# muhammadhasyim/cav-hoomd

Measured on AMD Instinct MI355X. Metric: cavity_force_evals_per_sec, higher is better.
Workload: dtype f64; 1 GPU; config3/config5: 1e6 diatomic particles + photon, finite-q start, g=1e-3, omegac=2000cm^-1; one independent replica per GPU (seed = rank+1); ring of 7 trajectory frames (HBM-cold); N_particles=1000001, frames=7, primed_frames=7, replicas=1, algorithmic_bytes_per_eval=92000092, layout=HOOMD AoS (Scalar4 pos/force, int3 image)

## Files before the change

### cav-hoomd_amd/csrc/cavmd_capi.hip

```cpp
#include <hip/hip_runtime.h>
#include <hip/hip_ext.h>

#include <math.h>
#include <stdio.h>
#include <stdlib.h>
#include <string.h>

#include <algorithm>
#include <new>
#include <vector>

#include "cavmd.h"
#include "cavmd_kernels.hpp"
#include "cavmd_host_support.hpp"

using namespace cavmd;

namespace
{
constexpr int kReduceBlock = 256;
constexpr int kReduceUnroll = 2;
constexpr int kFinalizeBlock = 256;
constexpr int kMapBlock = 256;
constexpr int kMapUnroll = 4;
constexpr int kMaxBlocksPerCU = 16;
constexpr int kEventsPerSlot = 6;
constexpr int kProfileSlots = 512;
constexpr size_t kMaxSamples = 4096;
constexpr int kSmallBlock = 256;
constexpr int kSmallSystemMaxN = 1024;
constexpr size_t kNtStoreMinN = 200000;
constexpr size_t kChargeTemporalMaxN = 25000000;
constexpr int kPersistBlock = 256;
constexpr size_t kPersistMaxLds = 156 * 1024;
constexpr uint64_t kSuspendFirst = 1ull << 16, kSuspendMax = 1ull << 31, kSuspendForever = ~0ull;
constexpr size_t kPersistSharedLds = 76 * 1024;
constexpr unsigned kResultHistory = 64;
constexpr unsigned kResultHistoryMax = 16384;

static_assert(sizeof(cavmd_double4) == 32, "Scalar4 layout");
static_assert(sizeof(cavmd_int3) == 12, "int3 layout");
static_assert(sizeof(cavmd_params) == 32, "params layout");
static_assert(sizeof(cavmd_result) == 192, "result layout");

struct HostControl
{
    HostResult fixed;
    unsigned sync_error;
    unsigned pad[63];
};
}

struct cavmd_workspace
{
    int device = -1;
    int num_cu = 0;
    char arch[64] = {0};
    size_t max_N = 0;
    unsigned max_parts = 0;
    DeviceArray<double> d_part;
    DeviceArray<int> d_ipart;
    DeviceArray<cavmd_result> d_result;
    MappedBlock<HostResult> h_ring;
    unsigned ring_depth = kResultHistory;
    uint64_t history_first = 1;
    MappedBlock<HostControl> h_ctl;
    hipStream_t last_stream = nullptr;
    bool computed = false;
    uint64_t sequence = 0;
    int reduce_blocks_per_cu = 1;
    int map_blocks_per_cu = 2;
    int map_nt_store = -1;
    int reduce_nt_load = -1;
    int fused_finalize = 1;
    int map_reverse = -1;
    int small_system_max_n = kSmallSystemMaxN;
    int reduce_unroll = -1;
    int persistent = -1;
    int rho_lane_particle = -1;
    int persistent_lds_kb = 0;
    int persistent_balanced = -1;
    DeviceArray<unsigned long long> d_granules;
    DeviceArray<unsigned> d_epoch;
    int debug_spin_limit = 0;
    int debug_late_block = -1;
    int debug_late_ticks = 0;
    int debug_silent_block = -1;
    int debug_skip_publish = 0;
    MappedBlock<HostResult> h_scratch;
    uint64_t suspend_until = 0;
    uint64_t suspend_backoff = kSuspendFirst;
    bool sync_state_dirty = false;
    bool sync_timeout_seen = false;
    bool captured = false;
    uint64_t captured_from = 0;
    bool profiling = false;
    std::vector<hipEvent_t> events;
    int pending = 0;
    std::vector<unsigned> slot_mask;
    double acc_ms[3] = {0, 0, 0};
    uint64_t acc_launches = 0;
    std::vector<float> samples;
    size_t n_k = 0;
    unsigned n_chunks = 0;
    unsigned rho_blocks = 0;
    DeviceArray<double> d_kvec, d_rho_part, d_rho;
    PinnedBlock<double> h_rho;
    hipStream_t rho_stream = nullptr;
    bool rho_computed = false;
    int rho_last_mapping = -1;
    int rho_last_blocks = -1;
    DeviceArray<double> d_mode;
    MappedBlock<HostMode> h_mode;
    uint64_t mode_sequence = 0;
    DeviceArray<double> d_fm_part;
    MappedBlock<HostScalar> h_fm;
    uint64_t fm_sequence = 0;
    DeviceArray<unsigned> d_fm_ticket;
    DeviceArray<BussiDevice> d_bussi;
    MappedBlock<HostBussi> h_bussi;
    uint64_t bussi_sequence = 0;
    uint64_t bussi_refused_seen = 0;
    hipStream_t bussi_stream = nullptr;
    unsigned bussi_batches = 0;
    unsigned recorders = 0;
    unsigned field_recorders = 0;
};

namespace
{
struct DeviceGuard
{
    int prev = -1;
    bool switched = false;
    explicit DeviceGuard(int dev)
    {
        if (hipGetDevice(&prev) == hipSuccess && prev != dev)
        {
            switched = (hipSetDevice(dev) == hipSuccess);
        }
    }
    ~DeviceGuard()
    {
        if (switched)
            (void)hipSetDevice(prev);
    }
};

inline int hip_status(hipError_t e)
{
    return e == hipSuccess ? CAVMD_OK : (int)e;
}

#define CAVMD_HIP_TRY(expr)              \
    do                                   \
    {                                    \
        hipError_t _e = (expr);          \
        if (_e != hipSuccess)            \
            return (int)_e;              \
    } while (0)

DeviceParams derive(const cavmd_params* p)
{
    DeviceParams d;
    d.g = p->couplstr;
    d.K = p->K;
    d.gK = p->couplstr / p->K;
    d.g2K = p->couplstr * p->couplstr / p->K;
    return d;
}

bool params_ok(const cavmd_params* p)
{
    return p && isfinite(p->omegac) && isfinite(p->couplstr) && isfinite(p->K) && isfinite(p->phmass) && p->K != 0.0;
}

int drain_profile(cavmd_workspace* ws)
{
    for (int s = 0; s < ws->pending; ++s)
    {
        hipEvent_t* ev = &ws->events[kEventsPerSlot * s];
        const unsigned used = ws->slot_mask[s];
        float sample[3] = {0.f, 0.f, 0.f};
        for (int k = 0; k < 3; ++k)
        {
            if (!(used & (1u << k)))
                continue;
            CAVMD_HIP_TRY(hipEventSynchronize(ev[2 * k + 1]));
            float ms = 0.f;
            CAVMD_HIP_TRY(hipEventElapsedTime(&ms, ev[2 * k], ev[2 * k + 1]));
            ws->acc_ms[k] += (double)ms;
            sample[k] = ms;
        }
        ws->acc_launches += 1;
        if (ws->samples.size() >= 3 * kMaxSamples)
            ws->samples.erase(ws->samples.begin(), ws->samples.begin() + 3);
        ws->samples.insert(ws->samples.end(), sample, sample + 3);
    }
    ws->pending = 0;
    return CAVMD_OK;
}

void note_capture(cavmd_workspace* ws, hipStream_t stream)
{
    if (!ws->captured && stream_capturing(stream))
    {
        ws->captured = true;
        ws->captured_from = ws->sequence;
    }
}

constexpr bool kPersistentAuto = true;
constexpr bool kPersistentBalancedAuto = false;

unsigned grid_for(size_t work_items, unsigned tile, int num_cu, int blocks_per_cu)
{
    size_t tiles = (work_items + tile - 1) / tile;
    size_t cap = (size_t)num_cu * (size_t)blocks_per_cu;
    size_t g = tiles < cap ? tiles : cap;
    return (unsigned)(g ? g : 1);
}

constexpr int kScaleBlocksPerCu = 4;
constexpr size_t kTicketBytes = 128;

int ensure_scalar_scratch(cavmd_workspace* ws)
{
    if (ws->d_fm_part.ptr)
        return CAVMD_OK;
    DeviceArray<double> part;
    MappedBlock<HostScalar> host;
    DeviceArray<unsigned> ticket;
    CAVMD_HIP_TRY(part.alloc(2 * (size_t)ws->max_parts + 1));
    CAVMD_HIP_TRY(host.alloc());
    CAVMD_HIP_TRY(ticket.alloc_zeroed(kTicketBytes / sizeof(unsigned)));
    ws->d_fm_part = std::move(part);
    ws->h_fm = std::move(host);
    ws->d_fm_ticket = std::move(ticket);
    return CAVMD_OK;
}

int wait_scalar(cavmd_workspace* ws, hipStream_t stream, double* out)
{
    const StampWait w = wait_for_stamp(&ws->h_fm.host->ready, ws->fm_sequence, stream);
    if (w.error != hipSuccess)
        return (int)w.error;
    if (!w.arrived)
    {
        (void)hipMemsetAsync(ws->d_fm_ticket.ptr, 0, kTicketBytes, stream);
        return (int)hipErrorLaunchFailure;
    }
    *out = ws->h_fm.host->value;
    return CAVMD_OK;
}

constexpr IntList<2, 1> kUnrolls;
constexpr IntList<0, 1, 2> kLoadPolicies;
constexpr IntList<2, 1, 0> kStorePolicies;

hipError_t allow_large_lds()
{
    hipError_t once = [] {
        hipError_t e = hipSuccess;
        const auto allow = [&e](auto kernel) {
            if (e == hipSuccess)
                e = hipFuncSetAttribute(reinterpret_cast<const void*>(kernel), hipFuncAttributeMaxDynamicSharedMemorySize,
                                        (int)kPersistMaxLds);
        };
        with_each_constant(kUnrolls, [&](auto u) {
            with_each_constant(kStorePolicies, [&](auto s) {
                allow(&cavity_persistent_kernel<kPersistBlock, decltype(u)::value, decltype(s)::value>);
            });
        });
#ifdef CAVMD_TEST_HOOKS
        with_each_constant(kUnrolls, [&](auto u) { allow(&cavity_persistent_kernel<kPersistBlock, decltype(u)::value, 0, true>); });
#endif
        return e;
    }();
    return once;
}

struct LaunchScope
{
    cavmd_workspace* ws;
    hipStream_t stream;
    hipEvent_t* ev = nullptr;
    unsigned used = 0;
    int status = CAVMD_OK;
    LaunchScope(cavmd_workspace* w, hipStream_t s) : ws(w), stream(s)
    {
        if (!ws->profiling)
            return;
        if (ws->pending == kProfileSlots)
            status = drain_profile(ws);
        if (status == CAVMD_OK)
            ev = &ws->events[kEventsPerSlot * ws->pending];
    }
    template <class K, class... Args>
    int launch_lds(int slot, size_t lds_bytes, K kernel, unsigned grid, unsigned block, Args... args)
    {
        if (ev)
        {
            hipExtLaunchKernelGGL(kernel, dim3(grid), dim3(block), lds_bytes, stream, ev[2 * slot], ev[2 * slot + 1], 0,
                                  args...);
            used |= 1u << slot;
        }
        else
            hipLaunchKernelGGL(kernel, dim3(grid), dim3(block), lds_bytes, stream, args...);
        return hip_status(hipGetLastError());
    }
    template <class K, class... Args>
    int launch(int slot, K kernel, unsigned grid, unsigned block, Args... args)
    {
        return launch_lds(slot, 0, kernel, grid, block, args...);
    }
    void commit()
    {
        if (ev)
        {
            ws->slot_mask[ws->pending] = used;
            ws->pending += 1;
        }
    }
};

enum class Layout
{
    aos,
    strided
};

enum class Path
{
    single_block,
    single_launch,
    two_launches,
    three_launches
};

struct EvalPlan
{
    Path path = Path::two_launches;
    Path multi_launch = Path::two_launches;
    int unroll = kReduceUnroll;
    unsigned g1 = 1, g2 = 1;
    int nt_load = 0;
    int nt_store = 0;
    unsigned lds_slots = 0;
    size_t lds_bytes = 0;
    bool balanced = false;
    bool map_reverse = false;
};

EvalPlan plan_evaluation(const cavmd_workspace& ws, size_t N, Layout layout)
{
    EvalPlan p;
    p.multi_launch = ws.fused_finalize ? Path::two_launches : Path::three_launches;
    p.path = p.multi_launch;
    if (layout == Layout::aos && ws.small_system_max_n > 0 && N <= (size_t)ws.small_system_max_n)
    {
        p.path = Path::single_block;
        return p;
    }
    p.unroll = kReduceUnroll;
    while (p.unroll > 1 && N / ((size_t)kReduceBlock * p.unroll) < (size_t)ws.num_cu * 5 / 4)
        p.unroll >>= 1;
    if (ws.reduce_unroll == 1 || ws.reduce_unroll == 2)
        p.unroll = ws.reduce_unroll;
    p.g1 = grid_for(N, kReduceBlock * p.unroll, ws.num_cu, ws.reduce_blocks_per_cu);
    if (layout == Layout::strided)
    {
        p.g2 = grid_for(N, kMapBlock * 4, ws.num_cu, ws.map_blocks_per_cu);
        return p;
    }
    p.g2 = grid_for(2 * N, kMapBlock * kMapUnroll, ws.num_cu, ws.map_blocks_per_cu);
    p.nt_store = ws.map_nt_store < 0 ? (N >= kNtStoreMinN ? 1 : 0) : ws.map_nt_store;
    p.nt_load = ws.reduce_nt_load < 0 ? (N <= kChargeTemporalMaxN ? 1 : 2) : ws.reduce_nt_load;
    p.map_reverse = ws.map_reverse < 0 ? (N > 2500000 && N <= 5000000) : (ws.map_reverse != 0);

    const size_t tile = (size_t)kReduceBlock * p.unroll;
    p.balanced = ws.persistent_balanced < 0 ? kPersistentBalancedAuto : (ws.persistent_balanced != 0);
    size_t slots;
    if (p.balanced)
    {
        const size_t units = (N + kWave - 1) / kWave;
        slots = (((units + p.g1 - 1) / p.g1) * kWave + tile - 1) / tile;
    }
    else
        slots = ((N + tile - 1) / tile + p.g1 - 1) / p.g1;
    size_t budget = kPersistMaxLds / (size_t)ws.reduce_blocks_per_cu - 1024;
    if (ws.persistent_lds_kb > 0 && (size_t)ws.persistent_lds_kb * 1024 < budget)
        budget = (size_t)ws.persistent_lds_kb * 1024;
    const size_t cap_slots = budget / (tile * sizeof(double));
    p.lds_slots = (unsigned)(slots < cap_slots ? slots : cap_slots);
    p.lds_bytes = p.lds_slots * tile * sizeof(double);
    const bool resident = p.g1 <= kMaxPersistGrid && ws.reduce_blocks_per_cu <= 4;
    if (resident
        && (ws.persistent > 0
            || (ws.persistent < 0 && slots <= cap_slots && p.lds_bytes <= kPersistSharedLds && kPersistentAuto)))
        p.path = Path::single_launch;
    return p;
}

int evaluation_enqueued(cavmd_workspace* ws, LaunchScope& ls, hipStream_t stream)
{
    ls.commit();
    ws->last_stream = stream;
    ws->computed = true;
    return CAVMD_OK;
}
}

extern "C"
{

cavmd_params cavmd_make_params(double omegac, double couplstr, double phmass)
{
    cavmd_params p;
    p.omegac = omegac;
    p.couplstr = couplstr;
    p.phmass = phmass;
    p.K = phmass * omegac * omegac;
    return p;
}

int cavmd_create(int device, size_t max_N, cavmd_workspace** out_ws)
{
    if (!out_ws)
        return CAVMD_ERR_INVALID_VALUE;
    *out_ws = nullptr;
    if (max_N > (size_t)INT_MAX)
        return CAVMD_ERR_CAPACITY;
    int count = 0;
    hipError_t e = hipGetDeviceCount(&count);
    if (e != hipSuccess || count <= 0)
        return CAVMD_ERR_NO_DEVICE;
    if (device < 0)
    {
        if (hipGetDevice(&device) != hipSuccess)
            return CAVMD_ERR_NO_DEVICE;
    }
    if (device >= count)
        return CAVMD_ERR_INVALID_VALUE;

    cavmd_workspace* ws = new (std::nothrow) cavmd_workspace();
    if (!ws)
        return (int)hipErrorOutOfMemory;
    ws->device = device;
    ws->max_N = max_N;
    if (const char* env = getenv("CAVMD_PERSISTENT"))
    {
        if (!strcmp(env, "0"))
            ws->persistent = 0;
        else if (!strcmp(env, "1"))
            ws->persistent = 1;
    }
    DeviceGuard guard(device);

    hipDeviceProp_t prop;
    e = hipGetDeviceProperties(&prop, device);
    if (e != hipSuccess)
    {
        delete ws;
        return (int)e;
    }
    ws->num_cu = prop.multiProcessorCount > 0 ? prop.multiProcessorCount : 256;
    strncpy(ws->arch, prop.gcnArchName, sizeof(ws->arch) - 1);
    ws->max_parts = (unsigned)(ws->num_cu * kMaxBlocksPerCU);

    e = ws->d_part.alloc((size_t)kNumPartDoubles * ws->max_parts);
    if (e == hipSuccess)
        e = ws->d_ipart.alloc((size_t)kNumPartInts * ws->max_parts);
    if (e == hipSuccess)
        e = ws->d_result.alloc_zeroed(1);
    if (e == hipSuccess)
        e = ws->d_granules.alloc_zeroed((size_t)2 * kGranulesPerRecord * kMaxPersistGrid);
    if (e == hipSuccess)
        e = ws->d_epoch.alloc(4);
    if (e == hipSuccess)
    {
        const unsigned init[4] = {1u, 0u, 0u, 0u};
        e = hipMemcpy(ws->d_epoch.ptr, init, sizeof(init), hipMemcpyHostToDevice);
    }
    if (e == hipSuccess)
        e = allow_large_lds();
    if (e == hipSuccess)
        e = ws->h_ring.alloc(ws->ring_depth);
    if (e == hipSuccess)
        e = ws->h_ctl.alloc();
    if (e != hipSuccess)
    {
        delete ws;
        return (int)e;
    }
    *out_ws = ws;
    return CAVMD_OK;
}

int cavmd_destroy(cavmd_workspace* ws)
{
    if (!ws)
        return CAVMD_OK;
    if (ws->bussi_batches != 0)
        return CAVMD_ERR_INVALID_VALUE;
    if (ws->recorders != 0)
        return CAVMD_ERR_INVALID_VALUE;
    if (ws->field_recorders != 0)
        return CAVMD_ERR_INVALID_VALUE;
    DeviceGuard guard(ws->device);
    for (hipEvent_t ev : ws->events)
        (void)hipEventDestroy(ev);
    delete ws;
    return CAVMD_OK;
}

namespace
{
inline HostResult* host_block(cavmd_workspace* ws)
{
#ifdef CAVMD_TEST_HOOKS
    if (ws->debug_skip_publish && ws->h_scratch.dev)
        return ws->h_scratch.dev;
#endif
    if (ws->captured)
        return &ws->h_ctl.dev->fixed;
    return ws->h_ring.dev + ws->sequence % ws->ring_depth;
}

inline HostResult* ring_slot(cavmd_workspace* ws, uint64_t s)
{
    return ws->h_ring.host + s % ws->ring_depth;
}

inline HostResult* last_block(cavmd_workspace* ws)
{
    if (ws->captured)
        return __atomic_load_n(&ws->h_ctl.host->fixed.ready, __ATOMIC_ACQUIRE) ? &ws->h_ctl.host->fixed
                                                                               : ring_slot(ws, ws->captured_from);
    return ring_slot(ws, ws->sequence);
}

unsigned consume_sync_timeout(cavmd_workspace* ws)
{
    if (!ws->h_ctl.host || !__atomic_load_n(&ws->h_ctl.host->sync_error, __ATOMIC_ACQUIRE))
        return 0;
    if (!stream_capturing(ws->last_stream))
        (void)hipStreamSynchronize(ws->last_stream);
    const unsigned verdict = __atomic_load_n(&ws->h_ctl.host->sync_error, __ATOMIC_ACQUIRE);
    __atomic_store_n(&ws->h_ctl.host->sync_error, 0u, __ATOMIC_RELEASE);
    ws->sync_timeout_seen = true;
    ws->sync_state_dirty = true;
    if (verdict == kSyncRepaired)
    {
        if (ws->sequence - ws->suspend_until > ws->suspend_backoff)
            ws->suspend_backoff = kSuspendFirst;
        ws->suspend_until = ws->sequence + ws->suspend_backoff;
        ws->suspend_backoff = ws->suspend_backoff * 8 < kSuspendMax ? ws->suspend_backoff * 8 : kSuspendMax;
        return kSyncRepaired;
    }
    ws->suspend_until = kSuspendForever;
    ws->computed = false;
    return kSyncFailed;
}
}

int cavmd_compute_hoomd(cavmd_workspace* ws, void* stream_, size_t N, const cavmd_double4* d_pos, const double* d_charge,
                        const cavmd_int3* d_image, double Lx, double Ly, double Lz, int L_typeid,
                        const cavmd_params* params, cavmd_double4* d_force)
{
    if (!ws || !d_pos || !d_charge || !d_image || !d_force || !params)
        return CAVMD_ERR_INVALID_VALUE;
    if (((uintptr_t)d_pos & 15) || ((uintptr_t)d_force & 15) || ((uintptr_t)d_charge & 7) || ((uintptr_t)d_image & 3))
        return CAVMD_ERR_INVALID_VALUE;
    if (N == 0)
        return CAVMD_OK;
    if (N > ws->max_N)
        return CAVMD_ERR_CAPACITY;
    if (!params_ok(params))
        return CAVMD_ERR_BAD_PARAMS;
    if (consume_sync_timeout(ws) == kSyncFailed)
        return CAVMD_ERR_SYNC_TIMEOUT;

    hipStream_t stream = (hipStream_t)stream_;
    DeviceGuard guard(ws->device);
    note_capture(ws, stream);
    LaunchScope ls(ws, stream);
    if (ls.status != CAVMD_OK)
        return ls.status;

    AosInput in;
    in.pos2 = reinterpret_cast<const v2d*>(d_pos);
    in.charge = d_charge;
    in.image = reinterpret_cast<const int*>(d_image);
    Partials part {ws->d_part.ptr, ws->d_ipart.ptr, ws->max_parts};
    const unsigned n = (unsigned)N;
    const DeviceParams dp = derive(params);
    v2d* force2 = reinterpret_cast<v2d*>(d_force);
    cavmd_result* const d_result = ws->d_result.ptr;
    int st;

    EvalPlan plan = plan_evaluation(*ws, N, Layout::aos);
    if (plan.path == Path::single_launch && ws->sequence < ws->suspend_until)
        plan.path = plan.multi_launch;

    if (plan.path == Path::single_block)
    {
        ws->sequence += 1;
        st = ls.launch(0, cavity_small_system_kernel<kSmallBlock>, 1u, kSmallBlock, in, n, Lx, Ly, Lz, dp, L_typeid,
                       ws->sequence, d_result, host_block(ws), force2);
        return st != CAVMD_OK ? st : evaluation_enqueued(ws, ls, stream);
    }

    if (plan.path == Path::single_launch)
    {
        if (ws->sync_state_dirty)
        {
            CAVMD_HIP_TRY(hipMemsetAsync(ws->d_granules.ptr, 0, sizeof(unsigned long long) * 2 * kGranulesPerRecord * kMaxPersistGrid, stream));
            CAVMD_HIP_TRY(hipMemsetAsync(ws->d_epoch.ptr + 1, 0, 2 * sizeof(unsigned), stream));
            ws->sync_state_dirty = false;
        }
        ws->sequence += 1;
        const AosInputT<2> inx {in.pos2, in.charge, in.image};
        const SyncState sync {ws->d_granules.ptr, ws->d_epoch.ptr,
                              ws->debug_spin_limit > 0 ? (unsigned)ws->debug_spin_limit : kSpinLimit, ws->debug_late_block,
                              (unsigned)ws->debug_late_ticks, ws->debug_silent_block, &ws->h_ctl.dev->sync_error};
        const auto launch = [&](auto kernel) {
            return ls.launch_lds(0, plan.lds_bytes, kernel, plan.g1, kPersistBlock, inx, n, Lx, Ly, Lz, dp, L_typeid, sync,
                                 ws->sequence, d_result, host_block(ws), force2, plan.lds_slots, plan.balanced);
        };
#ifdef CAVMD_TEST_HOOKS
        if (ws->debug_late_block >= 0 || ws->debug_silent_block >= 0)
            st = with_constant(kUnrolls, plan.unroll, [&](auto u) {
                return launch(&cavity_persistent_kernel<kPersistBlock, decltype(u)::value, 0, true>);
            });
        else
#endif
            st = with_constant(kUnrolls, plan.unroll, [&](auto u) {
                return with_constant(kStorePolicies, plan.nt_store, [&](auto s) {
                    return launch(&cavity_persistent_kernel<kPersistBlock, decltype(u)::value, decltype(s)::value>);
                });
            });
        return st != CAVMD_OK ? st : evaluation_enqueued(ws, ls, stream);
    }

    st = with_constant(kUnrolls, plan.unroll, [&](auto u) {
        return with_constant(kLoadPolicies, plan.nt_load, [&](auto nt) {
            using Input = AosInputT<decltype(nt)::value>;
            return ls.launch(0, &dipole_partials_kernel<Input, kReduceBlock, decltype(u)::value, false>, plan.g1, kReduceBlock,
                             Input {in.pos2, in.charge, in.image}, n, Lx, Ly, Lz, L_typeid, part);
        });
    });
    if (st != CAVMD_OK)
        return st;

    ws->sequence += 1;
    if (plan.path == Path::two_launches)
    {
        st = with_constant(kStorePolicies, plan.nt_store, [&](auto s) {
            return ls.launch(2, &force_map_aos_fused_kernel<kMapBlock, kMapUnroll, decltype(s)::value>, plan.g2, kMapBlock, in, n,
                             plan.g1, Lx, Ly, Lz, dp, L_typeid, part, ws->sequence, d_result, host_block(ws), force2,
                             plan.map_reverse);
        });
    }
    else
    {
        st = ls.launch(1, finalize_kernel<AosInput, kFinalizeBlock>, 1u, kFinalizeBlock, in, n, plan.g1, Lx, Ly, Lz, dp, part,
                       ws->sequence, d_result, host_block(ws));
        if (st != CAVMD_OK)
            return st;
        const cavmd_result* res = d_result;
        st = with_constant(IntList<1, 0> {}, plan.nt_store != 0, [&](auto nts) {
            return ls.launch(2, &force_map_aos_kernel<kMapBlock, kMapUnroll, decltype(nts)::value != 0>, plan.g2, kMapBlock,
                             d_charge, in.pos2, n, params->couplstr, L_typeid, res, force2);
        });
    }
    return st != CAVMD_OK ? st : evaluation_enqueued(ws, ls, stream);
}

int cavmd_compute_soa(cavmd_workspace* ws, void* stream_, size_t N, const double* d_position, size_t position_stride,
                      const int32_t* d_typeid, size_t typeid_stride, const int32_t* d_image, size_t image_stride,
                      const double* d_charge, size_t charge_stride, double Lx, double Ly, double Lz, int L_typeid,
                      const cavmd_params* params, double* d_force, size_t force_stride, double* d_potential_energy,
                      size_t potential_energy_stride)
{
    if (!ws || !d_position || !d_typeid || !d_image || !d_charge || !d_force || !params)
        return CAVMD_ERR_INVALID_VALUE;
    if (position_stride < 24 || typeid_stride < 4 || image_stride < 12 || charge_stride < 8 || force_stride < 24
        || (d_potential_energy && potential_energy_stride < 8))
        return CAVMD_ERR_INVALID_VALUE;
    if (((uintptr_t)d_position & 7) || (position_stride & 7) || ((uintptr_t)d_charge & 7) || (charge_stride & 7)
        || ((uintptr_t)d_force & 7) || (force_stride & 7) || ((uintptr_t)d_typeid & 3) || (typeid_stride & 3)
        || ((uintptr_t)d_image & 3) || (image_stride & 3)
        || (d_potential_energy && (((uintptr_t)d_potential_energy & 7) || (potential_energy_stride & 7))))
        return CAVMD_ERR_INVALID_VALUE;
    if (N == 0)
        return CAVMD_OK;
    if (N > ws->max_N)
        return CAVMD_ERR_CAPACITY;
    if (!params_ok(params))
        return CAVMD_ERR_BAD_PARAMS;

    {
        const char* p0 = reinterpret_cast<const char*>(d_position);
        const char* f0 = reinterpret_cast<const char*>(d_force);
        if (position_stride == 32 && typeid_stride == 32 && reinterpret_cast<const char*>(d_typeid) == p0 + 24
            && image_stride == 12 && charge_stride == 8 && force_stride == 32 && d_potential_energy
            && potential_energy_stride == 32 && reinterpret_cast<const char*>(d_potential_energy) == f0 + 24
            && !((uintptr_t)p0 & 15) && !((uintptr_t)f0 & 15))
        {
            return cavmd_compute_hoomd(ws, stream_, N, reinterpret_cast<const cavmd_double4*>(d_position), d_charge,
                                       reinterpret_cast<const cavmd_int3*>(d_image), Lx, Ly, Lz, L_typeid, params,
                                       reinterpret_cast<cavmd_double4*>(d_force));
        }
    }

    hipStream_t stream = (hipStream_t)stream_;
    DeviceGuard guard(ws->device);
    note_capture(ws, stream);
    LaunchScope ls(ws, stream);
    if (ls.status != CAVMD_OK)
        return ls.status;

    StridedInput in;
    in.pos = reinterpret_cast<const char*>(d_position);
    in.tid = reinterpret_cast<const char*>(d_typeid);
    in.img = reinterpret_cast<const char*>(d_image);
    in.chg = reinterpret_cast<const char*>(d_charge);
    in.pos_stride = position_stride;
    in.tid_stride = typeid_stride;
    in.img_stride = image_stride;
    in.chg_stride = charge_stride;
    Partials part {ws->d_part.ptr, ws->d_ipart.ptr, ws->max_parts};
    const unsigned n = (unsigned)N;
    const DeviceParams dp = derive(params);
    cavmd_result* const d_result = ws->d_result.ptr;

    const EvalPlan plan = plan_evaluation(*ws, N, Layout::strided);
    int st = with_constant(kUnrolls, plan.unroll, [&](auto u) {
        return ls.launch(0, &dipole_partials_kernel<StridedInput, kReduceBlock, decltype(u)::value, false>, plan.g1, kReduceBlock,
                         in, n, Lx, Ly, Lz, L_typeid, part);
    });
    if (st != CAVMD_OK)
        return st;
    ws->sequence += 1;
    char* f_out = reinterpret_cast<char*>(d_force);
    char* pe_out = reinterpret_cast<char*>(d_potential_energy);
    if (plan.path == Path::two_launches)
    {
        st = ls.launch(2, force_map_strided_fused_kernel<kMapBlock>, plan.g2, kMapBlock, in, n, plan.g1, Lx, Ly, Lz, dp, L_typeid,
                       part, ws->sequence, d_result, host_block(ws), f_out, force_stride, pe_out, potential_energy_stride);
    }
    else
    {
        st = ls.launch(1, finalize_kernel<StridedInput, kFinalizeBlock>, 1u, kFinalizeBlock, in, n, plan.g1, Lx, Ly, Lz, dp, part,
                       ws->sequence, d_result, host_block(ws));
        if (st != CAVMD_OK)
            return st;
        const cavmd_result* res = d_result;
        st = ls.launch(2, force_map_strided_kernel<kMapBlock>, plan.g2, kMapBlock, in, n, params->couplstr, L_typeid, res, f_out,
                       force_stride, pe_out, potential_energy_stride);
    }
    return st != CAVMD_OK ? st : evaluation_enqueued(ws, ls, stream);
}

int cavmd_result_read(cavmd_workspace* ws, cavmd_result* out)
{
    if (!ws || !out)
        return CAVMD_ERR_INVALID_VALUE;
    if (!ws->computed)
        return CAVMD_ERR_NOT_COMPUTED;
    DeviceGuard guard(ws->device);
    bool published = true;
    if (ws->captured)
    {
        CAVMD_HIP_TRY(hipDeviceSynchronize());
    }
    else
    {
        const StampWait w = wait_for_stamp(&ring_slot(ws, ws->sequence)->ready, ws->sequence, ws->last_stream);
        if (w.error != hipSuccess)
            return (int)w.error;
        published = w.arrived;
    }
    if (consume_sync_timeout(ws) == kSyncFailed)
        return CAVMD_ERR_SYNC_TIMEOUT;
    if (!published)
    {
        ws->computed = false;
        return (int)hipErrorLaunchFailure;
    }
    memcpy(out, &last_block(ws)->result, sizeof(cavmd_result));
    return CAVMD_OK;
}

int cavmd_energies(cavmd_workspace* ws, double out[3])
{
    if (!ws || !out)
        return CAVMD_ERR_INVALID_VALUE;
    if (!ws->computed)
    {
        out[0] = out[1] = out[2] = 0.0;
        return CAVMD_OK;
    }
    cavmd_result r;
    int st = cavmd_result_read(ws, &r);
    if (st != CAVMD_OK)
        return st;
    out[0] = r.energy[0];
    out[1] = r.energy[1];
    out[2] = r.energy[2];
    return CAVMD_OK;
}

int cavmd_last_sequence(cavmd_workspace* ws, uint64_t* out)
{
    if (!ws || !out)
        return CAVMD_ERR_INVALID_VALUE;
    *out = ws->sequence;
    return CAVMD_OK;
}

int cavmd_result_at(cavmd_workspace* ws, uint64_t sequence, cavmd_result* out)
{
    if (!ws || !out)
        return CAVMD_ERR_INVALID_VALUE;
    if (ws->sequence == 0)
        return CAVMD_ERR_NOT_COMPUTED;
    if (ws->captured)
        return CAVMD_ERR_INVALID_VALUE;
    const uint64_t last = ws->sequence;
    if (sequence == 0 || sequence > last)
        return CAVMD_ERR_INVALID_VALUE;
    if (sequence < ws->history_first || last - sequence >= ws->ring_depth)
        return CAVMD_ERR_EXPIRED;
    DeviceGuard guard(ws->device);
    const HostResult* h = ring_slot(ws, sequence);
    const StampWait w = wait_for_stamp(&h->ready, sequence, ws->last_stream, [&] {
        for (uint64_t j = sequence + 1; j <= last; ++j)
            if (__atomic_load_n(&ring_slot(ws, j)->ready, __ATOMIC_ACQUIRE) == j)
                return true;
        return false;
    });
    if (w.error != hipSuccess)
        return (int)w.error;
    if (!w.arrived)
    {
        const uint64_t failed = __atomic_load_n(&h->failed, __ATOMIC_ACQUIRE);
        return failed == ((sequence << 2) | kSyncFailed) ? CAVMD_ERR_SYNC_TIMEOUT : (int)hipErrorLaunchFailure;
    }
    memcpy(out, &h->result, sizeof(cavmd_result));
    return CAVMD_OK;
}

int cavmd_energies_at(cavmd_workspace* ws, uint64_t sequence, double out[3])
{
    if (!ws || !out)
        return CAVMD_ERR_INVALID_VALUE;
    cavmd_result r;
    const int st = cavmd_result_at(ws, sequence, &r);
    if (st != CAVMD_OK)
        return st;
    out[0] = r.energy[0];
    out[1] = r.energy[1];
    out[2] = r.energy[2];
    return CAVMD_OK;
}

int cavmd_result_device_ptr(cavmd_workspace* ws, const cavmd_result** out)
{
    if (!ws || !out)
        return CAVMD_ERR_INVALID_VALUE;
    *out = ws->d_result.ptr;
    return CAVMD_OK;
}

int cavmd_set_wavevectors(cavmd_workspace* ws, size_t n_k, const double* h_wavevectors)
{
    if (!ws || !h_wavevectors || n_k == 0 || n_k > (size_t)1 << 20)
        return CAVMD_ERR_INVALID_VALUE;
    DeviceGuard guard(ws->device);
    ws->d_kvec.free();
    ws->d_rho_part.free();
    ws->d_rho.free();
    ws->h_rho.free();
    ws->rho_computed = false;
    ws->n_k = 0;
    const unsigned n_chunks = (unsigned)((n_k + kWave - 1) / kWave);
    const unsigned rho_blocks = (unsigned)ws->num_cu * 4;
    DeviceArray<double> kvec, rho_part, rho;
    PinnedBlock<double> h_rho;
    CAVMD_HIP_TRY(kvec.alloc(3 * n_k));
    CAVMD_HIP_TRY(rho_part.alloc(2 * kWave * (size_t)n_chunks * rho_blocks));
    CAVMD_HIP_TRY(rho.alloc(2 * n_k));
    CAVMD_HIP_TRY(h_rho.alloc(2 * n_k));
    CAVMD_HIP_TRY(hipMemcpy(kvec.ptr, h_wavevectors, sizeof(double) * 3 * n_k, hipMemcpyHostToDevice));
    ws->d_kvec = std::move(kvec);
    ws->d_rho_part = std::move(rho_part);
    ws->d_rho = std::move(rho);
    ws->h_rho = std::move(h_rho);
    ws->n_k = n_k;
    ws->n_chunks = n_chunks;
    ws->rho_blocks = rho_blocks;
    return CAVMD_OK;
}

int cavmd_density_field(cavmd_workspace* ws, void* stream_, size_t N, const double* d_position, size_t position_stride)
{
    if (!ws || !d_position || position_stride < 24 || (position_stride & 7) || ((uintptr_t)d_position & 7))
        return CAVMD_ERR_INVALID_VALUE;
    if (ws->n_k == 0)
        return CAVMD_ERR_NOT_COMPUTED;
    if (N > (size_t)INT_MAX)
        return CAVMD_ERR_CAPACITY;
    hipStream_t stream = (hipStream_t)stream_;
    DeviceGuard guard(ws->device);
    constexpr int kBlock = 1024;
    const size_t tiles = (N + kWave - 1) / kWave;
    unsigned gb;
    int lp = ws->rho_lane_particle;
    if (lp < 0)
        lp = (ws->n_k * 4 < (size_t)ws->n_chunks * kWave * 3) ? 3 : 0;
    if (lp)
    {
        constexpr int kLpBlock = 256;
        size_t g = (tiles + (kLpBlock / kWave) - 1) / (kLpBlock / kWave);
        if (g > ws->rho_blocks)
            g = ws->rho_blocks;
        gb = (unsigned)(g ? g : 1);
        with_constant(IntList<25, 10, 5> {}, lp == 1 ? 25 : lp == 2 ? 10 : 5, [&](auto kc) {
            constexpr int KC = decltype(kc)::value;
            hipLaunchKernelGGL((density_partials_lp_kernel<kLpBlock, KC>), dim3(gb, (unsigned)((ws->n_k + KC - 1) / KC)),
                               dim3(kLpBlock), 0, stream, reinterpret_cast<const char*>(d_position), position_stride, (unsigned)N,
                               ws->d_kvec.ptr, (unsigned)ws->n_k, make_sincos_coef(), ws->d_rho_part.ptr);
        });
// ... 93 lines not shown
                       reinterpret_cast<const v2d*>(d_net_force), reinterpret_cast<const v2d*>(d_vel), (unsigned)N,
                       ws->d_fm_part.ptr, ws->d_fm_ticket.ptr, d_out, ws->h_fm.dev, ws->fm_sequence);
    CAVMD_HIP_TRY(hipGetLastError());
    return wait_scalar(ws, stream, out);
}

int cavmd_kinetic_energy(cavmd_workspace* ws, void* stream_, const cavmd_double4* d_vel, const uint32_t* d_members,
                         size_t n_members, double* out)
{
    if (!ws || !d_vel || !out || ((uintptr_t)d_vel & 15) || ((uintptr_t)d_members & 3))
        return CAVMD_ERR_INVALID_VALUE;
    if (n_members > (size_t)INT_MAX)
        return CAVMD_ERR_CAPACITY;
    if (n_members == 0)
    {
        *out = 0.0;
        return CAVMD_OK;
    }
    hipStream_t stream = (hipStream_t)stream_;
    DeviceGuard guard(ws->device);
    {
        const int st0 = ensure_scalar_scratch(ws);
        if (st0 != CAVMD_OK)
            return st0;
    }
    constexpr int kBlock = 256, kUnroll = 4;
    const unsigned g = grid_for(n_members, kBlock * kUnroll, ws->num_cu, 1);
    double* d_out = ws->d_fm_part.ptr + 2 * (size_t)ws->max_parts;
    ws->fm_sequence += 1;
    hipLaunchKernelGGL((kinetic_fused_kernel<kBlock, kUnroll>), dim3(g), dim3(kBlock), 0, stream,
                       reinterpret_cast<const v2d*>(d_vel), d_members, (unsigned)n_members, ws->d_fm_part.ptr,
                       ws->d_fm_ticket.ptr, d_out, ws->h_fm.dev, ws->fm_sequence);
    CAVMD_HIP_TRY(hipGetLastError());
    return wait_scalar(ws, stream, out);
}

int cavmd_scale_velocities(cavmd_workspace* ws, void* stream_, cavmd_double4* d_vel, const uint32_t* d_members,
                           size_t n_members, double alpha)
{
    if (!ws || !d_vel || ((uintptr_t)d_vel & 15) || ((uintptr_t)d_members & 3))
        return CAVMD_ERR_INVALID_VALUE;
    if (n_members > (size_t)INT_MAX)
        return CAVMD_ERR_CAPACITY;
    if (n_members == 0)
        return CAVMD_OK;
    hipStream_t stream = (hipStream_t)stream_;
    DeviceGuard guard(ws->device);
    constexpr int kBlock = 256, kUnroll = 4;
    const unsigned g = grid_for(n_members, kBlock * kUnroll, ws->num_cu, kScaleBlocksPerCu);
    hipLaunchKernelGGL((scale_velocities_kernel<kBlock, kUnroll>), dim3(g), dim3(kBlock), 0, stream, reinterpret_cast<v2d*>(d_vel),
                       d_members, (unsigned)n_members, alpha);
    return hip_status(hipGetLastError());
}

int cavmd_bussi_rescale_factor(double K, double degrees_of_freedom, double deltaT, double set_T, double tau,
                               double normal_variate, double gamma_variate, double* alpha)
{
    if (!alpha)
        return CAVMD_ERR_INVALID_VALUE;
    const double c = (tau != 0.0) ? exp(-deltaT / tau) : 0.0;
    *alpha = bussi_alpha_from_c(K, degrees_of_freedom, c, set_T, normal_variate, gamma_variate);
    return CAVMD_OK;
}

int cavmd_bussi_step(cavmd_bussi_reservoir* state, double K_translational, double dof_translational, double K_rotational,
                     double dof_rotational, double deltaT, double set_T, double tau, const double variates[4],
                     double factors[2])
{
    if (!state || !variates || !factors)
        return CAVMD_ERR_INVALID_VALUE;
    if (deltaT == 0.0)
    {
        factors[0] = factors[1] = 1.0;
        return CAVMD_OK;
    }
    if ((dof_translational != 0 && K_translational == 0) || (dof_rotational != 0 && K_rotational == 0))
        return CAVMD_ERR_BAD_PARAMS;
    double at = 1.0, ar = 1.0;
    (void)cavmd_bussi_rescale_factor(K_translational, dof_translational, deltaT, set_T, tau, variates[0], variates[1], &at);
    (void)cavmd_bussi_rescale_factor(K_rotational, dof_rotational, deltaT, set_T, tau, variates[2], variates[3], &ar);
    const double delta_t = K_translational * (1.0 - at * at);
    const double delta_r = K_rotational * (1.0 - ar * ar);
    state->reservoir_translational += delta_t;
    state->reservoir_rotational += delta_r;
    state->instantaneous_translational = delta_t;
    state->instantaneous_rotational = delta_r;
    factors[0] = at;
    factors[1] = ar;
    return CAVMD_OK;
}

namespace
{
int ensure_bussi_state(cavmd_workspace* ws)
{
    if (ws->d_bussi.ptr)
        return CAVMD_OK;
    DeviceArray<BussiDevice> state;
    MappedBlock<HostBussi> host;
    CAVMD_HIP_TRY(state.alloc_zeroed(1));
    CAVMD_HIP_TRY(host.alloc());
    ws->d_bussi = std::move(state);
    ws->h_bussi = std::move(host);
    return CAVMD_OK;
}
}

int cavmd_bussi_step_device(cavmd_workspace* ws, void* stream_, cavmd_double4* d_vel, const uint32_t* d_members,
                            size_t n_members, double dof_translational, double deltaT, double set_T, double tau,
                            double normal_variate, double gamma_variate)
{
    if (!ws || !d_vel || ((uintptr_t)d_vel & 15) || ((uintptr_t)d_members & 3))
        return CAVMD_ERR_INVALID_VALUE;
    if (n_members > (size_t)INT_MAX)
        return CAVMD_ERR_CAPACITY;
    hipStream_t stream = (hipStream_t)stream_;
    if (capture_state(stream) != Capture::none)
        return CAVMD_ERR_INVALID_VALUE;
    if (deltaT == 0.0 || n_members == 0)
        return CAVMD_OK;
    DeviceGuard guard(ws->device);
    {
        int st0 = ensure_scalar_scratch(ws);
        if (st0 == CAVMD_OK)
            st0 = ensure_bussi_state(ws);
        if (st0 != CAVMD_OK)
            return st0;
    }
    constexpr int kBlock = 256, kUnroll = 4;
    BussiStepArgs a;
    a.dof = dof_translational;
    a.c = (tau != 0.0) ? exp(-deltaT / tau) : 0.0;
    a.set_T = set_T;
    a.normal_variate = normal_variate;
    a.gamma_variate = gamma_variate;
    const unsigned g = grid_for(n_members, kBlock * kUnroll, ws->num_cu, 1);
    ws->bussi_sequence += 1;
    ws->bussi_stream = stream;
    hipLaunchKernelGGL((kinetic_partials_kernel<kBlock, kUnroll>), dim3(g), dim3(kBlock), 0, stream,
                       reinterpret_cast<const v2d*>(d_vel), d_members, (unsigned)n_members, ws->d_fm_part.ptr);
    CAVMD_HIP_TRY(hipGetLastError());
    const unsigned g2 = grid_for(n_members, kBlock * kUnroll, ws->num_cu, kScaleBlocksPerCu);
    hipLaunchKernelGGL((bussi_rescale_fused_kernel<kBlock, kUnroll>), dim3(g2), dim3(kBlock), 0, stream,
                       reinterpret_cast<v2d*>(d_vel), d_members, (unsigned)n_members, ws->d_fm_part.ptr, g, a, ws->d_bussi.ptr,
                       ws->h_bussi.dev, ws->bussi_sequence);
    return hip_status(hipGetLastError());
}

int cavmd_bussi_device_read(cavmd_workspace* ws, cavmd_bussi_device_state* out)
{
    if (!ws || !out)
        return CAVMD_ERR_INVALID_VALUE;
    memset(out, 0, sizeof(*out));
    if (!ws->d_bussi.ptr || ws->bussi_sequence == 0)
        return CAVMD_OK;
    DeviceGuard guard(ws->device);
    const StampWait w = wait_for_stamp(&ws->h_bussi.host->ready, ws->bussi_sequence, ws->bussi_stream);
    if (w.error != hipSuccess)
        return (int)w.error;
    if (!w.arrived)
        return (int)hipErrorLaunchFailure;
    const BussiDevice s = ws->h_bussi.host->state;
    out->reservoir_translational = s.reservoir;
    out->instantaneous_translational = s.instantaneous;
    out->last_alpha = s.alpha;
    out->last_kinetic_energy = s.kinetic;
    out->steps = s.steps;
    out->refused = s.errors;
    if (s.errors != ws->bussi_refused_seen)
    {
        ws->bussi_refused_seen = s.errors;
        return CAVMD_ERR_BAD_PARAMS;
    }
    return CAVMD_OK;
}

int cavmd_bussi_device_reset(cavmd_workspace* ws, void* stream_)
{
    if (!ws)
        return CAVMD_ERR_INVALID_VALUE;
    if (!ws->d_bussi.ptr)
        return CAVMD_OK;
    hipStream_t stream = (hipStream_t)stream_;
    DeviceGuard guard(ws->device);
    cavmd_bussi_device_state unused;
    const int st = cavmd_bussi_device_read(ws, &unused);
    if (st != CAVMD_OK && st != CAVMD_ERR_BAD_PARAMS)
        return st;
    CAVMD_HIP_TRY(hipMemsetAsync(ws->d_bussi.ptr, 0, sizeof(BussiDevice), stream));
    memset(&ws->h_bussi.host->state, 0, sizeof(BussiDevice));
    ws->bussi_refused_seen = 0;
    return CAVMD_OK;
}

int cavmd_profile_enable(cavmd_workspace* ws, int on)
{
    if (!ws)
        return CAVMD_ERR_INVALID_VALUE;
    DeviceGuard guard(ws->device);
    if (on && ws->events.empty())
    {
        ws->events.resize(kEventsPerSlot * kProfileSlots);
        ws->slot_mask.assign(kProfileSlots, 0);
        for (size_t i = 0; i < ws->events.size(); ++i)
        {
            hipError_t e = hipEventCreate(&ws->events[i]);
            if (e != hipSuccess)
            {
                for (size_t j = 0; j < i; ++j)
                    (void)hipEventDestroy(ws->events[j]);
                ws->events.clear();
                return (int)e;
            }
        }
    }
    if (!on && ws->pending)
    {
        int st = drain_profile(ws);
        if (st != CAVMD_OK)
            return st;
    }
    ws->profiling = on != 0;
    return CAVMD_OK;
}

int cavmd_profile_read(cavmd_workspace* ws, double ms[3], uint64_t* launches)
{
    if (!ws || !ms || !launches)
        return CAVMD_ERR_INVALID_VALUE;
    DeviceGuard guard(ws->device);
    int st = drain_profile(ws);
    if (st != CAVMD_OK)
        return st;
    for (int k = 0; k < 3; ++k)
    {
        ms[k] = ws->acc_ms[k];
        ws->acc_ms[k] = 0.0;
    }
    *launches = ws->acc_launches;
    ws->acc_launches = 0;
    ws->samples.clear();
    return CAVMD_OK;
}

int cavmd_profile_samples(cavmd_workspace* ws, double* out, size_t cap, size_t* n)
{
    if (!ws || !out || !n)
        return CAVMD_ERR_INVALID_VALUE;
    DeviceGuard guard(ws->device);
    int st = drain_profile(ws);
    if (st != CAVMD_OK)
        return st;
    const size_t have = ws->samples.size() / 3;
    const size_t take = have < cap ? have : cap;
    const size_t first = have - take;
    for (size_t i = 0; i < 3 * take; ++i)
        out[i] = (double)ws->samples[3 * first + i];
    *n = take;
    return CAVMD_OK;
}

namespace
{
int resize_history(cavmd_workspace* ws, unsigned depth)
{
    if (stream_capturing(ws->last_stream))
        return CAVMD_ERR_INVALID_VALUE;
    DeviceGuard guard(ws->device);
    if (ws->sequence)
        CAVMD_HIP_TRY(hipStreamSynchronize(ws->last_stream));
    MappedBlock<HostResult> ring;
    CAVMD_HIP_TRY(ring.alloc(depth));
    const uint64_t keep = ws->captured ? ws->captured_from : ws->sequence;
    if (keep)
        memcpy(ring.host + keep % depth, ring_slot(ws, keep), sizeof(HostResult));
    ws->h_ring = std::move(ring);
    ws->ring_depth = depth;
    ws->history_first = ws->sequence ? ws->sequence : 1;
    return CAVMD_OK;
}

struct TunableRow
{
    const char* name;
    int cavmd_workspace::*member;
    int lo, hi;
};
const TunableRow kTunables[] = {
    {"reduce_blocks_per_cu", &cavmd_workspace::reduce_blocks_per_cu, 1, kMaxBlocksPerCU},
    {"map_blocks_per_cu", &cavmd_workspace::map_blocks_per_cu, 1, kMaxBlocksPerCU},
    {"map_nt_store", &cavmd_workspace::map_nt_store, -1, 2},
    {"reduce_nt_load", &cavmd_workspace::reduce_nt_load, -1, 2},
    {"fused_finalize", &cavmd_workspace::fused_finalize, 0, 1},
    {"map_reverse", &cavmd_workspace::map_reverse, -1, 1},
    {"small_system_max_n", &cavmd_workspace::small_system_max_n, 0, 1 << 20},
    {"rho_lane_particle", &cavmd_workspace::rho_lane_particle, -1, 3},
    {"persistent_lds_kb", &cavmd_workspace::persistent_lds_kb, 0, 156},
    {"persistent_balanced", &cavmd_workspace::persistent_balanced, -1, 1},
#ifdef CAVMD_TEST_HOOKS
    {"debug_spin_limit", &cavmd_workspace::debug_spin_limit, 0, INT_MAX},
    {"debug_late_block", &cavmd_workspace::debug_late_block, -1, (int)kMaxPersistGrid - 1},
    {"debug_late_ticks", &cavmd_workspace::debug_late_ticks, 0, 100000000},
    {"debug_silent_block", &cavmd_workspace::debug_silent_block, -1, (int)kMaxPersistGrid - 1},
#endif
};

const TunableRow* find_tunable(const char* name)
{
    for (const TunableRow& row : kTunables)
        if (!strcmp(name, row.name))
            return &row;
    return nullptr;
}
}

int cavmd_set_tunable(cavmd_workspace* ws, const char* name, int value)
{
    if (!ws || !name)
        return CAVMD_ERR_INVALID_VALUE;
    if (const TunableRow* row = find_tunable(name))
    {
        if (value < row->lo || value > row->hi)
            return CAVMD_ERR_INVALID_VALUE;
        ws->*(row->member) = value;
        return CAVMD_OK;
    }
    if (!strcmp(name, "result_history"))
    {
        if (value < 2 || value > (int)kResultHistoryMax)
            return CAVMD_ERR_INVALID_VALUE;
        return resize_history(ws, (unsigned)value);
    }
    if (!strcmp(name, "persistent"))
    {
        if (value < -1 || value > 1)
            return CAVMD_ERR_INVALID_VALUE;
        ws->persistent = value;
        ws->suspend_until = 0;
        ws->suspend_backoff = kSuspendFirst;
        return CAVMD_OK;
    }
    if (!strcmp(name, "reduce_unroll"))
    {
        if (value != -1 && value != 1 && value != 2)
            return CAVMD_ERR_INVALID_VALUE;
        ws->reduce_unroll = value;
        return CAVMD_OK;
    }
#ifdef CAVMD_TEST_HOOKS
    if (!strcmp(name, "debug_suspend_first"))
    {
        if (value < 1)
            return CAVMD_ERR_INVALID_VALUE;
        ws->suspend_backoff = (uint64_t)value;
        return CAVMD_OK;
    }
    if (!strcmp(name, "debug_skip_publish"))
    {
        if (value < 0 || value > 1)
            return CAVMD_ERR_INVALID_VALUE;
        if (value && !ws->h_scratch.host)
        {
            DeviceGuard guard(ws->device);
            CAVMD_HIP_TRY(ws->h_scratch.alloc());
        }
        ws->debug_skip_publish = value;
        return CAVMD_OK;
    }
#endif
    if (!strcmp(name, "sync_timeout_seen"))
    {
#ifdef CAVMD_TEST_HOOKS
        if (value < 0 || value > 2)
            return CAVMD_ERR_INVALID_VALUE;
        if (value)
            __atomic_store_n(&ws->h_ctl.host->sync_error, value == 2 ? kSyncRepaired : kSyncFailed, __ATOMIC_RELEASE);
        else
            ws->sync_timeout_seen = false;
#else
        if (value != 0)
            return CAVMD_ERR_INVALID_VALUE;
        ws->sync_timeout_seen = false;
#endif
        return CAVMD_OK;
    }
    return CAVMD_ERR_INVALID_VALUE;
}

int cavmd_get_tunable(cavmd_workspace* ws, const char* name, int* value)
{
    if (!ws || !name || !value)
        return CAVMD_ERR_INVALID_VALUE;
    if (const TunableRow* row = find_tunable(name))
        *value = ws->*(row->member);
    else if (!strcmp(name, "result_history"))
        *value = (int)ws->ring_depth;
    else if (!strcmp(name, "persistent"))
        *value = ws->persistent;
    else if (!strcmp(name, "reduce_unroll"))
        *value = ws->reduce_unroll;
    else if (!strcmp(name, "sync_timeout_seen"))
        *value = ws->sync_timeout_seen ? 1 : 0;
    else if (!strcmp(name, "persistent_suspended"))
        *value = ws->suspend_until == kSuspendForever ? 2 : (ws->sequence < ws->suspend_until ? 1 : 0);
    else if (!strcmp(name, "rho_last_mapping"))
        *value = ws->rho_last_mapping;
    else if (!strcmp(name, "rho_last_blocks"))
        *value = ws->rho_last_blocks;
#ifdef CAVMD_TEST_HOOKS
    else if (!strcmp(name, "debug_skip_publish"))
        *value = ws->debug_skip_publish;
    else if (!strcmp(name, "test_hooks"))
        *value = 1;
#else
    else if (!strcmp(name, "test_hooks"))
        *value = 0;
#endif
    else
        return CAVMD_ERR_INVALID_VALUE;
    return CAVMD_OK;
}

int cavmd_device_info(cavmd_workspace* ws, int* device, int* compute_units, char* arch_name, size_t arch_name_len)
{
    if (!ws)
        return CAVMD_ERR_INVALID_VALUE;
    if (device)
        *device = ws->device;
    if (compute_units)
        *compute_units = ws->num_cu;
    if (arch_name && arch_name_len)
    {
        strncpy(arch_name, ws->arch, arch_name_len - 1);
        arch_name[arch_name_len - 1] = 0;
    }
    return CAVMD_OK;
}

const char* cavmd_error_string(int status)
{
    switch (status)
    {
    case CAVMD_OK:
        return "success";
    case CAVMD_ERR_INVALID_VALUE:
        return "invalid value (null or misaligned pointer, bad stride or size)";
    case CAVMD_ERR_NO_DEVICE:
        return "no HIP device available (this library has no CPU fallback)";
    case CAVMD_ERR_CAPACITY:
        return "N exceeds the workspace capacity";
    case CAVMD_ERR_BAD_PARAMS:
        return "bad cavity parameters (K == 0 or non-finite)";
    case CAVMD_ERR_NOT_COMPUTED:
        return "no evaluation has been enqueued on this workspace yet";
    case CAVMD_ERR_EXPIRED:
        return "that evaluation's result slot has been reused: read it sooner or raise the \"result_history\" tunable";
    case CAVMD_ERR_SYNC_TIMEOUT:
        return "a single-launch evaluation was starved (its workgroups were not resident together) and could not be completed; "
               "forces of that evaluation are NaN";
    default:
        break;
    }
    if (status > 0)
        return hipGetErrorString((hipError_t)status);
    return "unknown cavmd status";
}

int cavmd_version(void)
{
    return CAVMD_VERSION_MAJOR * 1000 + CAVMD_VERSION_MINOR;
}

}

#include "cavmd_item_table.hpp"

namespace
{
constexpr int kBatchBlock = kSmallBlock;
constexpr size_t kBatchRingMaxBytes = (size_t)64 << 20;
static_assert(sizeof(cavmd_batch_item) == 128, "batch item layout");

BatchRow batch_row(const cavmd_batch_item& it)
{
    BatchRow r;
    memset(&r, 0, sizeof(r));
    r.pos2 = reinterpret_cast<const v2d*>(it.d_pos);
    r.charge = it.d_charge;
    r.image = reinterpret_cast<const int*>(it.d_image);
    r.force2 = reinterpret_cast<v2d*>(it.d_force);
    r.Lx = it.Lx; r.Ly = it.Ly; r.Lz = it.Lz;
    if (it.N)
        r.prm = derive(&it.params);
    r.N = it.N;
    r.L_typeid = it.L_typeid;
    return r;
}
}

struct cavmd_batch : ItemTable<cavmd_batch_item, BatchRow>
{
    unsigned depth = 0;
    DeviceArray<cavmd_result> d_result;
    MappedBlock<HostResult> h_ring;
    uint64_t sequence = 0;
    bool captured = false;

    cavmd_batch() : ItemTable(cavmd_batch_item_check, [](const cavmd_batch_item& it) { return it.N; }, batch_row) {}
};

namespace
{
inline const HostResult* batch_slot(const cavmd_batch* b, uint64_t s)
{
    return b->h_ring.host + (s % b->depth) * b->n;
}
}

extern "C"
{

int cavmd_batch_item_check(const cavmd_batch_item* it)
{
    if (!it)
        return CAVMD_ERR_INVALID_VALUE;
    for (int k = 0; k < 4; ++k)
        if (it->reserved[k] != 0)
            return CAVMD_ERR_INVALID_VALUE;
    if (it->N != 0 && (!it->d_pos || !it->d_charge || !it->d_image || !it->d_force))
        return CAVMD_ERR_INVALID_VALUE;
    if (((uintptr_t)it->d_pos & 15) || ((uintptr_t)it->d_force & 15) || ((uintptr_t)it->d_charge & 7)
        || ((uintptr_t)it->d_image & 3))
        return CAVMD_ERR_INVALID_VALUE;
    if (it->N == 0)
        return CAVMD_OK;
    if (it->N > CAVMD_BATCH_MAX_ITEM_N)
        return CAVMD_ERR_CAPACITY;
    if (!params_ok(&it->params))
        return CAVMD_ERR_BAD_PARAMS;
    return CAVMD_OK;
}

int cavmd_batch_create(cavmd_workspace* ws, size_t n_items, const cavmd_batch_item* h_items, int history_depth,
                       cavmd_batch** out)
{
    if (!out)
        return CAVMD_ERR_INVALID_VALUE;
    *out = nullptr;
    if (!ws || !h_items || n_items == 0 || n_items > CAVMD_BATCH_MAX_ITEMS || history_depth < 2
        || history_depth > (int)kResultHistoryMax)
        return CAVMD_ERR_INVALID_VALUE;
    const int st = check_items(h_items, n_items, cavmd_batch_item_check);
    if (st != CAVMD_OK)
        return st;
    const size_t ring_blocks = (size_t)history_depth * n_items;
    if (ring_blocks * sizeof(HostResult) > kBatchRingMaxBytes)
        return CAVMD_ERR_CAPACITY;

    cavmd_batch* b = new (std::nothrow) cavmd_batch();
    if (!b)
        return (int)hipErrorOutOfMemory;
    b->adopt(ws->device, h_items, n_items);
    b->depth = (unsigned)history_depth;

    DeviceGuard guard(b->device);
    hipError_t e = b->upload();
    if (e == hipSuccess)
        e = b->d_result.alloc_zeroed(n_items);
    if (e == hipSuccess)
        e = b->h_ring.alloc(ring_blocks);
    if (e != hipSuccess)
    {
        cavmd_batch_destroy(b);
        return (int)e;
    }
    *out = b;
    return CAVMD_OK;
}

int cavmd_batch_destroy(cavmd_batch* b)
{
    if (!b)
        return CAVMD_OK;
    DeviceGuard guard(b->device);
    b->quiesce_and_free();
    delete b;
    return CAVMD_OK;
}

int cavmd_batch_set_items(cavmd_batch* b, size_t first, size_t count, const cavmd_batch_item* h_items)
{
    return b ? b->set_items(first, count, h_items) : CAVMD_ERR_INVALID_VALUE;
}

int cavmd_batch_compute(cavmd_batch* b, void* stream_)
{
    if (!b)
        return CAVMD_ERR_INVALID_VALUE;
    hipStream_t stream = (hipStream_t)stream_;
    DeviceGuard guard(b->device);
    if (!b->captured && stream_capturing(stream))
        b->captured = true;
    b->sequence += 1;
    HostResult* host = b->h_ring.dev + (b->sequence % b->depth) * b->n;
    hipLaunchKernelGGL(cavity_batch_kernel<kBatchBlock>, dim3((unsigned)b->n), dim3(kBatchBlock), 0, stream, b->d_rows,
                       b->d_order, b->sequence, b->d_result.ptr, host);
// ... 688 lines not shown
```

### cav-hoomd_amd/csrc/cavmd_force_kernels.hpp

```cpp
#pragma once

#include "cavmd_reduce.hpp"

#pragma clang fp contract(off)

namespace cavmd
{

template <int NT>
struct AosInputT
{
    const v2d* __restrict__ pos2;
    const double* __restrict__ charge;
    const int* __restrict__ image;

    struct Raw
    {
        v2d xy, zw;
        double c;
        int ix, iy, iz;
    };
    __device__ __forceinline__ Raw load(size_t i) const
    {
        Raw r;
// ... 5 lines not shown
            r.c = (NT == 2) ? __builtin_nontemporal_load(charge + i) : charge[i];
            r.ix = __builtin_nontemporal_load(im + 0);
            r.iy = __builtin_nontemporal_load(im + 1);
            r.iz = __builtin_nontemporal_load(im + 2);
        }
        else
        {
            r.xy = pos2[2 * i];
            r.zw = pos2[2 * i + 1];
            r.c = charge[i];
            r.ix = im[0];
            r.iy = im[1];
            r.iz = im[2];
        }
        return r;
    }
    static __device__ __forceinline__ double x(const Raw& r) { return r.xy.x; }
    static __device__ __forceinline__ double y(const Raw& r) { return r.xy.y; }
    static __device__ __forceinline__ double z(const Raw& r) { return r.zw.x; }
    static __device__ __forceinline__ int tag(const Raw& r) { return __double2loint(r.zw.y); }
};
typedef AosInputT<0> AosInput;

struct StridedInput
{
    const char* __restrict__ pos;
    const char* __restrict__ tid;
    const char* __restrict__ img;
    const char* __restrict__ chg;
    size_t pos_stride, tid_stride, img_stride, chg_stride;

    struct Raw
    {
        double px, py, pz, c;
        int ix, iy, iz, t;
    };
    __device__ __forceinline__ Raw load(size_t i) const
    {
        Raw r;
        const double* p = reinterpret_cast<const double*>(pos + i * pos_stride);
        r.px = __builtin_nontemporal_load(p + 0);
        r.py = __builtin_nontemporal_load(p + 1);
        r.pz = __builtin_nontemporal_load(p + 2);
        r.c = *reinterpret_cast<const double*>(chg + i * chg_stride);
        const int* im = reinterpret_cast<const int*>(img + i * img_stride);
        r.ix = __builtin_nontemporal_load(im + 0);
        r.iy = __builtin_nontemporal_load(im + 1);
        r.iz = __builtin_nontemporal_load(im + 2);
        r.t = __builtin_nontemporal_load(reinterpret_cast<const int*>(tid + i * tid_stride));
        return r;
    }
    static __device__ __forceinline__ double x(const Raw& r) { return r.px; }
    static __device__ __forceinline__ double y(const Raw& r) { return r.py; }
    static __device__ __forceinline__ double z(const Raw& r) { return r.pz; }
    static __device__ __forceinline__ int tag(const Raw& r) { return r.t; }
};

struct DeviceParams
{
    double g;
    double K;
    double gK;
    double g2K;
};

struct PhotonRow
{
    double x, y, z;
    int ix, iy, iz;
};
template <class Input>
__device__ __forceinline__ PhotonRow photon_row(const Input& in, size_t i)
{
    const typename Input::Raw r = in.load(i);
    PhotonRow p;
    p.x = Input::x(r); p.y = Input::y(r); p.z = Input::z(r);
    p.ix = r.ix; p.iy = r.iy; p.iz = r.iz;
    return p;
}

struct Partials
{
    double* d;
    int* i;
    unsigned stride;
};

template <class Input, int UNROLL>
struct TileRegs
{
    typename Input::Raw raw[UNROLL];
};

template <class Input, int BLOCK, int UNROLL>
__device__ __forceinline__ void tile_load(const Input& in, size_t base, TileRegs<Input, UNROLL>& r)
{
#pragma unroll
    for (int u = 0; u < UNROLL; ++u)
        r.raw[u] = in.load(base + (size_t)u * BLOCK);
}

template <class Input, int BLOCK, int UNROLL>
__device__ __forceinline__ void tile_accumulate(const TileRegs<Input, UNROLL>& r, size_t base, double Lx, double Ly,
                                                double Lz, int L_typeid, Accum& acc)
{
    bool isL[UNROLL];
    bool any = false;
#pragma unroll
    for (int u = 0; u < UNROLL; ++u)
    {
        isL[u] = (Input::tag(r.raw[u]) == L_typeid);
        any = any || isL[u];
    }
    if (!__any(any))
    {
#pragma unroll
        for (int u = 0; u < UNROLL; ++u)
        {
            const double c = r.raw[u].c;
            dd_acc(acc.hx, acc.lx, c * (Input::x(r.raw[u]) + (double)r.raw[u].ix * Lx));
            dd_acc(acc.hy, acc.ly, c * (Input::y(r.raw[u]) + (double)r.raw[u].iy * Ly));
            dd_acc(acc.hz, acc.lz, c * (Input::z(r.raw[u]) + (double)r.raw[u].iz * Lz));
        }
    }
    else
    {
#pragma unroll
        for (int u = 0; u < UNROLL; ++u)
        {
            const double rx = Input::x(r.raw[u]) + (double)r.raw[u].ix * Lx;
            const double ry = Input::y(r.raw[u]) + (double)r.raw[u].iy * Ly;
            const double rz = Input::z(r.raw[u]) + (double)r.raw[u].iz * Lz;
            acc.add((unsigned)(base + (size_t)u * BLOCK), rx, ry, rz, r.raw[u].c, Input::tag(r.raw[u]), L_typeid);
        }
    }
}

template <class Input, int BLOCK, int UNROLL, bool PIPE>
__global__ __launch_bounds__(BLOCK) void dipole_partials_kernel(Input in, unsigned N, double Lx, double Ly, double Lz,
                                                                int L_typeid, Partials part)
{
    constexpr unsigned TILE = BLOCK * UNROLL;
    Accum acc;
    const unsigned full_tiles = N / TILE;
    const unsigned G = gridDim.x;
    if (!PIPE)
    {
        for (unsigned t = blockIdx.x; t < full_tiles; t += G)
        {
            const size_t base = (size_t)t * TILE + threadIdx.x;
            TileRegs<Input, UNROLL> A;
            tile_load<Input, BLOCK, UNROLL>(in, base, A);
            __builtin_amdgcn_sched_barrier(0);
            tile_accumulate<Input, BLOCK, UNROLL>(A, base, Lx, Ly, Lz, L_typeid, acc);
        }
    }
    else
    {
        TileRegs<Input, UNROLL> A, B;
        unsigned t = blockIdx.x;
        if (t < full_tiles)
            tile_load<Input, BLOCK, UNROLL>(in, (size_t)t * TILE + threadIdx.x, A);
        while (t < full_tiles)
        {
            if (t + G < full_tiles)
                tile_load<Input, BLOCK, UNROLL>(in, (size_t)(t + G) * TILE + threadIdx.x, B);
            __builtin_amdgcn_sched_barrier(0);
            tile_accumulate<Input, BLOCK, UNROLL>(A, (size_t)t * TILE + threadIdx.x, Lx, Ly, Lz, L_typeid, acc);
            t += G;
            if (t >= full_tiles)
                break;
            if (t + G < full_tiles)
                tile_load<Input, BLOCK, UNROLL>(in, (size_t)(t + G) * TILE + threadIdx.x, A);
            __builtin_amdgcn_sched_barrier(0);
            tile_accumulate<Input, BLOCK, UNROLL>(B, (size_t)t * TILE + threadIdx.x, Lx, Ly, Lz, L_typeid, acc);
            t += G;
        }
    }
    if (blockIdx.x == full_tiles % G)
    {
        const size_t base = (size_t)full_tiles * TILE + threadIdx.x;
#pragma unroll
        for (int u = 0; u < UNROLL; ++u)
        {
            const size_t i = base + (size_t)u * BLOCK;
            if (i < N)
            {
                const typename Input::Raw r = in.load(i);
                const double rx = Input::x(r) + (double)r.ix * Lx;
                const double ry = Input::y(r) + (double)r.iy * Ly;
                const double rz = Input::z(r) + (double)r.iz * Lz;
                acc.add((unsigned)i, rx, ry, rz, r.c, Input::tag(r), L_typeid);
            }
        }
    }
    acc = block_reduce<BLOCK>(acc);
    if (threadIdx.x == 0)
    {
        const unsigned b = blockIdx.x, s = part.stride;
        part.d[0 * s + b] = acc.hx; part.d[1 * s + b] = acc.lx;
        part.d[2 * s + b] = acc.hy; part.d[3 * s + b] = acc.ly;
        part.d[4 * s + b] = acc.hz; part.d[5 * s + b] = acc.lz;
        part.d[6 * s + b] = acc.sx; part.d[7 * s + b] = acc.sy; part.d[8 * s + b] = acc.sz;
        part.i[0 * s + b] = acc.lmin;
        part.i[1 * s + b] = acc.lcnt;
    }
}

struct Scalars
{
    double d[3], dlo[3], q[3], Dq[2], e[3], f[3], dtot[3];
    int photon, nL;
};

template <class Input>
__device__ __forceinline__ Scalars scalars_from_total(Accum acc, const PhotonRow guess, const Input& in,
                                                      unsigned N, double Lx, double Ly, double Lz,
                                                      const DeviceParams& prm, bool want_energies)
{
    Scalars sc;
    dd_norm(acc.hx, acc.lx);
    dd_norm(acc.hy, acc.ly);
    if (want_energies)
        dd_norm(acc.hz, acc.lz);
    double dx = acc.hx, dy = acc.hy, dz = acc.hz;
    sc.dtot[0] = sc.dtot[1] = sc.dtot[2] = 0.0;
    if (want_energies)
    {
        double th = acc.hx, tl = acc.lx;
        dd_acc(th, tl, acc.sx);
        sc.dtot[0] = th + tl;
        th = acc.hy; tl = acc.ly;
        dd_acc(th, tl, acc.sy);
        sc.dtot[1] = th + tl;
        th = acc.hz; tl = acc.lz;
        dd_acc(th, tl, acc.sz);
        sc.dtot[2] = th + tl;
    }
    const int photon = (acc.lmin == INT_MAX) ? -1 : acc.lmin;
    const double g = prm.g, K = prm.K;
    double qx = 0.0, qy = 0.0, qz = 0.0, eh = 0.0, ec = 0.0, ed = 0.0, Dqx = 0.0, Dqy = 0.0, fx = 0.0, fy = 0.0, fz = 0.0;
    if (threadIdx.x == 0)
    {
        if (photon >= 0)
        {
            double px = guess.x, py = guess.y, pz = guess.z;
            int pix = guess.ix, piy = guess.iy, piz = guess.iz;
            if ((unsigned)photon != N - 1)
            {
                const PhotonRow r = photon_row(in, (size_t)photon);
                px = r.x; py = r.y; pz = r.z;
                pix = r.ix; piy = r.iy; piz = r.iz;
            }
            qx = px + (double)pix * Lx;
            qy = py + (double)piy * Ly;
            qz = pz + (double)piz * Lz;
            if (acc.lcnt > 1)
            {
                const double pc = in.load((size_t)photon).c;
                dx += acc.sx - pc * qx;
                dy += acc.sy - pc * qy;
                dz += acc.sz - pc * qz;
            }
            if (want_energies)
            {
                eh = 0.5 * K * (qx * qx + qy * qy + qz * qz);
                ec = g * (dx * qx + dy * qy + 0.0 * 0.0);
                ed = 0.5 * prm.g2K * (dx * dx + dy * dy + 0.0 * 0.0);
            }
            Dqx = qx + prm.gK * dx;
            Dqy = qy + prm.gK * dy;
            fx = -K * qx - g * dx;
            fy = -K * qy - g * dy;
            fz = -K * qz - g * 0.0;
        }
        else
        {
            dx = dy = dz = 0.0;
            acc.lx = acc.ly = acc.lz = 0.0;
        }
    }
    CAVMD_STAMP(4);
    sc.d[0] = dx; sc.d[1] = dy; sc.d[2] = dz;
    sc.dlo[0] = acc.lx; sc.dlo[1] = acc.ly; sc.dlo[2] = acc.lz;
    sc.q[0] = qx; sc.q[1] = qy; sc.q[2] = qz;
    sc.Dq[0] = Dqx; sc.Dq[1] = Dqy;
    sc.e[0] = eh; sc.e[1] = ec; sc.e[2] = ed;
    sc.f[0] = fx; sc.f[1] = fy; sc.f[2] = fz;
    sc.photon = photon;
    sc.nL = acc.lcnt;
    return sc;
}

template <class Input, int BLOCK>
__device__ __forceinline__ Scalars reduce_partials_and_finalize(const Input& in, unsigned N, unsigned nparts, double Lx,
                                                                double Ly, double Lz, const DeviceParams& prm,
                                                                const Partials& part, bool want_energies)
{
    CAVMD_STAMP(0);
    const PhotonRow guess = photon_row(in, (size_t)(N - 1));

    Accum acc;
    const unsigned s = part.stride;
    constexpr int BATCH = 4;
    for (unsigned base = 0; base < nparts; base += BATCH * BLOCK)
    {
        Accum o[BATCH];
#pragma unroll
        for (int j = 0; j < BATCH; ++j)
        {
            const unsigned p = base + j * BLOCK + threadIdx.x;
            if (p < nparts)
            {
                o[j].hx = part.d[0 * s + p]; o[j].lx = part.d[1 * s + p];
                o[j].hy = part.d[2 * s + p]; o[j].ly = part.d[3 * s + p];
                o[j].hz = part.d[4 * s + p]; o[j].lz = part.d[5 * s + p];
                o[j].sx = part.d[6 * s + p]; o[j].sy = part.d[7 * s + p]; o[j].sz = part.d[8 * s + p];
                o[j].lmin = part.i[0 * s + p];
                o[j].lcnt = part.i[1 * s + p];
            }
        }
#pragma unroll
        for (int j = 0; j < BATCH; ++j)
            if (base + j * BLOCK < nparts)
                acc.merge(o[j]);
    }
    CAVMD_STAMP(1);
    if (BLOCK == 256 && nparts <= 256)
    {
        __shared__ double s_gd[16][kNumPartDoubles];
        __shared__ int s_gi[16][kNumPartInts];
        acc = row_fold16(acc);
        CAVMD_STAMP(2);
        if ((threadIdx.x & 15) == 0)
        {
            const int gidx = threadIdx.x >> 4;
            s_gd[gidx][0] = acc.hx; s_gd[gidx][1] = acc.lx; s_gd[gidx][2] = acc.hy; s_gd[gidx][3] = acc.ly;
            s_gd[gidx][4] = acc.hz; s_gd[gidx][5] = acc.lz; s_gd[gidx][6] = acc.sx; s_gd[gidx][7] = acc.sy;
            s_gd[gidx][8] = acc.sz;
            s_gi[gidx][0] = acc.lmin;
            s_gi[gidx][1] = acc.lcnt;
        }
        __syncthreads();
        if (threadIdx.x < kWave)
        {
            Accum o;
            if (threadIdx.x < (nparts + 15) / 16)
            {
                const int gidx = threadIdx.x;
                o.hx = s_gd[gidx][0]; o.lx = s_gd[gidx][1]; o.hy = s_gd[gidx][2]; o.ly = s_gd[gidx][3];
                o.hz = s_gd[gidx][4]; o.lz = s_gd[gidx][5]; o.sx = s_gd[gidx][6]; o.sy = s_gd[gidx][7];
                o.sz = s_gd[gidx][8];
                o.lmin = s_gi[gidx][0];
                o.lcnt = s_gi[gidx][1];
            }
            Accum t;
            t.merge(o);
            acc = row_fold16(t);
        }
        CAVMD_STAMP(3);
    }
    else
        acc = block_reduce<BLOCK>(acc);
    return scalars_from_total<Input>(acc, guess, in, N, Lx, Ly, Lz, prm, want_energies);
}

__device__ __forceinline__ void write_result(cavmd_result* __restrict__ res, const Scalars& sc, unsigned N,
                                             unsigned nparts, uint64_t sequence)
{
#pragma unroll
    for (int k = 0; k < 3; ++k)
    {
        res->dipole[k] = sc.d[k];
        res->q[k] = sc.q[k];
        res->energy[k] = sc.e[k];
        res->photon_force[k] = sc.f[k];
        res->dipole_lo[k] = sc.dlo[k];
        res->total_dipole[k] = sc.dtot[k];
    }
    res->Dq[0] = sc.Dq[0];
    res->Dq[1] = sc.Dq[1];
    res->photon_idx = sc.photon;
    res->n_photon_typed = sc.nL;
    res->n_particles = N;
    res->n_partials = nparts;
    res->sequence = sequence;
    res->reserved = 0.0;
}

struct HostResult
{
    cavmd_result result;
    uint64_t ready;
    uint64_t failed;
    unsigned char pad[48];
};
static_assert(sizeof(HostResult) == 256, "one result slot = 256 bytes");
__device__ __forceinline__ void publish_to_host(HostResult* __restrict__ host, const Scalars& sc, unsigned N,
                                                unsigned nparts, uint64_t sequence)
{
    write_result(&host->result, sc, N, nparts, sequence);
    __hip_atomic_store(&host->ready, sequence, __ATOMIC_RELEASE, __HIP_MEMORY_SCOPE_SYSTEM);
}

template <class Input, int BLOCK>
__global__ __launch_bounds__(BLOCK) void finalize_kernel(Input in, unsigned N, unsigned nparts, double Lx, double Ly,
                                                         double Lz, DeviceParams prm, Partials part, uint64_t sequence,
                                                         cavmd_result* __restrict__ res, HostResult* __restrict__ res_host)
{
    const Scalars sc = reduce_partials_and_finalize<Input, BLOCK>(in, N, nparts, Lx, Ly, Lz, prm, part, true);
    if (threadIdx.x == 0)
    {
        write_result(res, sc, N, nparts, sequence);
        publish_to_host(res_host, sc, N, nparts, sequence);
    }
}

template <int NT>
__device__ __forceinline__ void store_chunk(v2d* p, v2d v)
{
    if (NT == 2)
    {
        asm volatile("global_store_dwordx4 %0, %1, off sc1\n\ts_nop 1" : : "v"(p), "v"(v) : "memory");
    }
    else if (NT == 1)
        __builtin_nontemporal_store(v, p);
    else
        *p = v;
}

struct MapScalars
{
    double Dqx, Dqy, Fx, Fy, Fz;
    int photon, nL;
};

template <int BLOCK, int UNROLL, int NT, bool PRE>
__device__ __forceinline__ void force_map_body(const MapScalars m, const double* __restrict__ charge,
                                               const v2d* __restrict__ pos2, unsigned N, double g, int L_typeid,
                                               v2d* __restrict__ force2, const double (&c_first)[UNROLL],
                                               bool reverse = false)
{
    constexpr unsigned TILE = BLOCK * UNROLL;
    const double ng = -g;
    const size_t nchunks = 2 * (size_t)N;
    const size_t pchunk = m.photon >= 0 ? 2 * (size_t)m.photon : ~(size_t)0;
    const unsigned full_tiles = (unsigned)(nchunks / TILE);
    const bool odd = threadIdx.x & 1;
    const v2d zero = {0.0, 0.0};

    if (m.photon < 0)
    {
        for (size_t k = (size_t)blockIdx.x * BLOCK + threadIdx.x; k < nchunks; k += (size_t)gridDim.x * BLOCK)
            store_chunk<NT>(force2 + k, zero);
        return;
    }

    if (m.nL <= 1)
    {
        const unsigned count = blockIdx.x < full_tiles ? (full_tiles - blockIdx.x + gridDim.x - 1) / gridDim.x : 0;
        for (unsigned j = 0; j < count; ++j)
        {
            const unsigned t = blockIdx.x + (reverse ? count - 1 - j : j) * gridDim.x;
            const size_t base = (size_t)t * TILE + threadIdx.x;
            double c[UNROLL];
            if (PRE && j == 0)
            {
#pragma unroll
                for (int u = 0; u < UNROLL; ++u)
                    c[u] = c_first[u];
            }
            else
            {
#pragma unroll
                for (int u = 0; u < UNROLL; ++u)
                    c[u] = charge[(base + (size_t)u * BLOCK) >> 1];
            }
#pragma unroll
            for (int u = 0; u < UNROLL; ++u)
            {
                const size_t k = base + (size_t)u * BLOCK;
                const double s = ng * c[u];
                v2d v = {s * m.Dqx, s * m.Dqy};
                v = odd ? zero : v;
                if ((k | 1) == (pchunk | 1))
                    v = odd ? (v2d) {m.Fz, 0.0} : (v2d) {m.Fx, m.Fy};
                store_chunk<NT>(force2 + k, v);
            }
        }
        if (blockIdx.x == full_tiles % gridDim.x)
        {
            const size_t base = (size_t)full_tiles * TILE + threadIdx.x;
#pragma unroll
            for (int u = 0; u < UNROLL; ++u)
            {
                const size_t k = base + (size_t)u * BLOCK;
                if (k < nchunks)
                {
                    const double s = ng * charge[k >> 1];
                    v2d v = {s * m.Dqx, s * m.Dqy};
                    v = odd ? zero : v;
                    if ((k | 1) == (pchunk | 1))
                        v = odd ? (v2d) {m.Fz, 0.0} : (v2d) {m.Fx, m.Fy};
                    store_chunk<NT>(force2 + k, v);
                }
            }
        }
        return;
    }

    for (size_t k = (size_t)blockIdx.x * BLOCK + threadIdx.x; k < nchunks; k += (size_t)gridDim.x * BLOCK)
    {
        const size_t p = k >> 1;
        const int tag = __double2loint(pos2[2 * p + 1].y);
        const double s = ng * charge[p];
        v2d v = {s * m.Dqx, s * m.Dqy};
        v = (odd || tag == L_typeid) ? zero : v;
        if ((k | 1) == (pchunk | 1))
            v = odd ? (v2d) {m.Fz, 0.0} : (v2d) {m.Fx, m.Fy};
        store_chunk<NT>(force2 + k, v);
    }
}

template <int BLOCK, int UNROLL, int NT>
__global__ __launch_bounds__(BLOCK) void force_map_aos_kernel(const double* __restrict__ charge,
                                                              const v2d* __restrict__ pos2,
                                                              unsigned N, double g, int L_typeid,
                                                              const cavmd_result* __restrict__ res, v2d* __restrict__ force2)
{
    MapScalars m;
    m.Dqx = res->Dq[0]; m.Dqy = res->Dq[1];
    m.Fx = res->photon_force[0]; m.Fy = res->photon_force[1]; m.Fz = res->photon_force[2];
    m.photon = res->photon_idx;
    m.nL = res->n_photon_typed;
    const double none[UNROLL] = {};
    force_map_body<BLOCK, UNROLL, NT, false>(m, charge, pos2, N, g, L_typeid, force2, none);
}

template <int BLOCK, int UNROLL, int NT>
__global__ __launch_bounds__(BLOCK) void force_map_aos_fused_kernel(AosInput in, unsigned N, unsigned nparts, double Lx,
                                                                    double Ly, double Lz, DeviceParams prm, int L_typeid,
                                                                    Partials part, uint64_t sequence,
                                                                    cavmd_result* __restrict__ res,
                                                                    HostResult* __restrict__ res_host,
                                                                    v2d* __restrict__ force2, bool reverse)
{
    __shared__ double s_m[5];
    __shared__ int s_mi[2];
    double c_first[UNROLL] = {};
    {
        constexpr unsigned TILE = BLOCK * UNROLL;
        const unsigned full_tiles = (unsigned)((2 * (size_t)N) / TILE);
        if (blockIdx.x < full_tiles)
        {
            const unsigned count = (full_tiles - blockIdx.x + gridDim.x - 1) / gridDim.x;
            const unsigned t0 = blockIdx.x + (reverse ? count - 1 : 0) * gridDim.x;
            const size_t base = (size_t)t0 * TILE + threadIdx.x;
#pragma unroll
            for (int u = 0; u < UNROLL; ++u)
                c_first[u] = in.charge[(base + (size_t)u * BLOCK) >> 1];
        }
    }
    const Scalars sc = reduce_partials_and_finalize<AosInput, BLOCK>(in, N, nparts, Lx, Ly, Lz, prm, part, blockIdx.x == 0);
    if (threadIdx.x == 0)
    {
        s_m[0] = sc.Dq[0]; s_m[1] = sc.Dq[1]; s_m[2] = sc.f[0]; s_m[3] = sc.f[1]; s_m[4] = sc.f[2];
        s_mi[0] = sc.photon;
        s_mi[1] = sc.nL;
        if (blockIdx.x == 0)
        {
            write_result(res, sc, N, nparts, sequence);
            publish_to_host(res_host, sc, N, nparts, sequence);
        }
    }
    __syncthreads();
    MapScalars m;
    m.Dqx = s_m[0]; m.Dqy = s_m[1]; m.Fx = s_m[2]; m.Fy = s_m[3]; m.Fz = s_m[4];
    m.photon = s_mi[0];
    m.nL = s_mi[1];
    force_map_body<BLOCK, UNROLL, NT, true>(m, in.charge, in.pos2, N, prm.g, L_typeid, force2, c_first, reverse);
}

constexpr int kSmallSystemLdsCharges = 4096;

template <int BLOCK>
__global__ __launch_bounds__(BLOCK) void cavity_small_system_kernel(AosInput in, unsigned N, double Lx, double Ly, double Lz,
                                                                    DeviceParams prm, int L_typeid, uint64_t sequence,
                                                                    cavmd_result* __restrict__ res,
                                                                    HostResult* __restrict__ res_host,
                                                                    v2d* __restrict__ force2)
{
#include "cavmd_small_system_body.hpp"
}

template <int BLOCK, int UNROLL>
__device__ __forceinline__ void force_map_strided_body(const MapScalars m, const StridedInput& in, unsigned N, double g,
                                                       int L_typeid, char* __restrict__ force, size_t force_stride,
                                                       char* __restrict__ pe, size_t pe_stride)
{
    const double ng = -g;
    constexpr size_t TILE = (size_t)BLOCK * UNROLL;
    const size_t tiles = ((size_t)N + TILE - 1) / TILE;
    for (size_t t = blockIdx.x; t < tiles; t += gridDim.x)
    {
        const size_t base = t * TILE + threadIdx.x;
        double c[UNROLL];
#pragma unroll
        for (int u = 0; u < UNROLL; ++u)
        {
            const size_t i = base + (size_t)u * BLOCK;
            c[u] = (m.photon >= 0 && i < N) ? *reinterpret_cast<const double*>(in.chg + i * in.chg_stride) : 0.0;
        }
#pragma unroll
        for (int u = 0; u < UNROLL; ++u)
        {
            const size_t i = base + (size_t)u * BLOCK;
            if (i >= N)
                continue;
            double fx = 0.0, fy = 0.0, fz = 0.0;
            if (m.photon >= 0)
            {
                const double s = ng * c[u];
                fx = s * m.Dqx;
                fy = s * m.Dqy;
                if (m.nL > 1 && *reinterpret_cast<const int*>(in.tid + i * in.tid_stride) == L_typeid)
                {
                    fx = 0.0;
                    fy = 0.0;
                }
                if ((int)i == m.photon)
                {
                    fx = m.Fx;
                    fy = m.Fy;
                    fz = m.Fz;
                }
            }
            double* f = reinterpret_cast<double*>(force + i * force_stride);
            __builtin_nontemporal_store(fx, f + 0);
            __builtin_nontemporal_store(fy, f + 1);
            __builtin_nontemporal_store(fz, f + 2);
            if (pe)
                __builtin_nontemporal_store(0.0, reinterpret_cast<double*>(pe + i * pe_stride));
        }
    }
}

template <int BLOCK>
__global__ __launch_bounds__(BLOCK) void force_map_strided_kernel(StridedInput in, unsigned N, double g, int L_typeid,
                                                                  const cavmd_result* __restrict__ res,
                                                                  char* __restrict__ force, size_t force_stride,
                                                                  char* __restrict__ pe, size_t pe_stride)
{
    MapScalars m;
    m.Dqx = res->Dq[0]; m.Dqy = res->Dq[1];
    m.Fx = res->photon_force[0]; m.Fy = res->photon_force[1]; m.Fz = res->photon_force[2];
    m.photon = res->photon_idx;
    m.nL = res->n_photon_typed;
    force_map_strided_body<BLOCK, 4>(m, in, N, g, L_typeid, force, force_stride, pe, pe_stride);
}

template <int BLOCK>
__global__ __launch_bounds__(BLOCK) void force_map_strided_fused_kernel(StridedInput in, unsigned N, unsigned nparts,
                                                                        double Lx, double Ly, double Lz, DeviceParams prm,
                                                                        int L_typeid, Partials part, uint64_t sequence,
                                                                        cavmd_result* __restrict__ res,
                                                                        HostResult* __restrict__ res_host,
// ... 28 lines not shown
```

### cav-hoomd_amd/csrc/cavmd_persistent_kernel.hpp

```cpp
#pragma once

#include "cavmd_force_kernels.hpp"

#pragma clang fp contract(off)

#ifndef CAVMD_PSTAMP
#define CAVMD_PSTAMP(k)
#endif

namespace cavmd
{

constexpr int kGranulesPerRecord = 2 * kNumPartDoubles + kNumPartInts;
constexpr unsigned kSpinLimit = 1000000;
constexpr unsigned kRepairRounds = 4096;

constexpr int kGroup = 16;
constexpr unsigned kMaxPersistGrid = kGroup * kGroup;
#ifndef CAVMD_GROUP_COPIES
#define CAVMD_GROUP_COPIES 8
#endif
#ifndef CAVMD_POLL_SLEEP
#define CAVMD_POLL_SLEEP 1
#endif
constexpr unsigned kGroupCopies = CAVMD_GROUP_COPIES;

struct SyncState
{
    unsigned long long* granules;
    unsigned* epoch;
    unsigned spin_limit;
    int late_block;
    unsigned late_ticks;
    int silent_block;
    unsigned* sync_error;
};
constexpr unsigned kSyncFailed = 1u;
constexpr unsigned kSyncRepaired = 2u;

__device__ __forceinline__ unsigned long long granule_load(const unsigned long long* g)
{
    return __hip_atomic_load(g, __ATOMIC_RELAXED, __HIP_MEMORY_SCOPE_AGENT);
}

__device__ __forceinline__ void record_to_lds(unsigned* s_rec, const Accum& a)
{
    const double d[kNumPartDoubles] = {a.hx, a.lx, a.hy, a.ly, a.hz, a.lz, a.sx, a.sy, a.sz};
#pragma unroll
    for (int i = 0; i < kNumPartDoubles; ++i)
    {
        s_rec[2 * i] = (unsigned)__double2loint(d[i]);
        s_rec[2 * i + 1] = (unsigned)__double2hiint(d[i]);
    }
    s_rec[2 * kNumPartDoubles] = (unsigned)a.lmin;
    s_rec[2 * kNumPartDoubles + 1] = (unsigned)a.lcnt;
}

__device__ __forceinline__ void record_from_lds(const unsigned* w, Accum& o)
{
    o.hx = __hiloint2double((int)w[1], (int)w[0]);   o.lx = __hiloint2double((int)w[3], (int)w[2]);
    o.hy = __hiloint2double((int)w[5], (int)w[4]);   o.ly = __hiloint2double((int)w[7], (int)w[6]);
    o.hz = __hiloint2double((int)w[9], (int)w[8]);   o.lz = __hiloint2double((int)w[11], (int)w[10]);
    o.sx = __hiloint2double((int)w[13], (int)w[12]); o.sy = __hiloint2double((int)w[15], (int)w[14]);
    o.sz = __hiloint2double((int)w[17], (int)w[16]);
    o.lmin = (int)w[18];
    o.lcnt = (int)w[19];
}

__device__ __forceinline__ void publish_record(unsigned long long* slab, unsigned slab_records, unsigned copies, unsigned rec,
                                               unsigned tag, const Accum& a, unsigned* s_pub)
{
    const unsigned lane = threadIdx.x;
    if (lane == 0)
        record_to_lds(s_pub, a);
    const unsigned field = lane % kGranulesPerRecord, copy0 = lane / kGranulesPerRecord;
    const unsigned long long granule = ((unsigned long long)tag << 32) | s_pub[field];
    for (unsigned c = copy0; c < copies && copy0 < 3; c += 3)
        __hip_atomic_store(slab + ((size_t)c * slab_records + rec) * kGranulesPerRecord + field, granule, __ATOMIC_RELAXED,
                           __HIP_MEMORY_SCOPE_AGENT);
}

__device__ __forceinline__ bool gather_records(const unsigned long long* slab, unsigned first, unsigned count, unsigned tag,
                                               unsigned* s_words, Accum& o, unsigned max_rounds, int own_slot,
                                               const Accum& own, const unsigned* giveups = nullptr)
{
    constexpr int ROUNDS = (kGroup * kGranulesPerRecord + kWave - 1) / kWave;
    const unsigned lane = threadIdx.x;
    const unsigned total = count * kGranulesPerRecord;
    const unsigned long long* g = slab + (size_t)first * kGranulesPerRecord;
    unsigned long long x[ROUNDS];
    for (unsigned spins = 1;; ++spins)
    {
        const unsigned gone = giveups ? __hip_atomic_load(giveups, __ATOMIC_RELAXED, __HIP_MEMORY_SCOPE_AGENT) : 0u;
#pragma unroll
        for (int j = 0; j < ROUNDS; ++j)
        {
            const unsigned i = j * kWave + lane;
            x[j] = granule_load(g + (i < total ? i : total - 1));
        }
        bool ok = true;
#pragma unroll
        for (int j = 0; j < ROUNDS; ++j)
        {
            const unsigned i = j * kWave + lane;
            const bool mine = own_slot >= 0 && (i < total ? i : total - 1) / kGranulesPerRecord == (unsigned)own_slot;
            ok = ok && (mine || (unsigned)(x[j] >> 32) == tag);
        }
        if (gone != 0)
            return false;
        if (__all(ok))
            break;
        if (spins >= max_rounds)
            return false;
        if (CAVMD_POLL_SLEEP > 0)
            __builtin_amdgcn_s_sleep(CAVMD_POLL_SLEEP);
    }
#pragma unroll
    for (int j = 0; j < ROUNDS; ++j)
        if ((unsigned)(j * kWave) + lane < total)
            s_words[j * kWave + lane] = (unsigned)x[j];
    if (own_slot >= 0 && lane == 0)
        record_to_lds(s_words + own_slot * kGranulesPerRecord, own);
    if (lane < count)
        record_from_lds(s_words + lane * kGranulesPerRecord, o);
    return true;
}

struct BlockRange
{
    size_t first, step, tail_base;
    unsigned nfull, tail_count;
};
template <unsigned TILE>
__device__ __forceinline__ BlockRange block_range(unsigned N, unsigned G, unsigned b, int balanced)
{
    BlockRange r;
    if (balanced == 2)
    {
        const unsigned rounds = (N / TILE) / G;
        const size_t done = (size_t)rounds * G * TILE;
        const unsigned long long U = ((unsigned long long)(N - done) + kWave - 1) / kWave;
        const size_t s = done + (size_t)(U * b / G) * kWave;
        size_t e = done + (size_t)(U * (b + 1) / G) * kWave;
        e = e < N ? e : N;
        r.first = (size_t)b * TILE;
        r.step = (size_t)G * TILE;
        r.nfull = rounds;
        r.tail_base = s;
        r.tail_count = (unsigned)(e > s ? e - s : 0);
    }
    else if (balanced)
    {
        const unsigned long long U = ((unsigned long long)N + kWave - 1) / kWave;
        const size_t s = (size_t)(U * b / G) * kWave;
        size_t e = (size_t)(U * (b + 1) / G) * kWave;
        e = e < N ? e : N;
        const size_t n = e > s ? e - s : 0;
        r.first = s;
        r.step = TILE;
        r.nfull = (unsigned)(n / TILE);
        r.tail_base = s + (size_t)r.nfull * TILE;
        r.tail_count = (unsigned)(n - (size_t)r.nfull * TILE);
    }
    else
    {
        const unsigned full_tiles = N / TILE;
        r.first = (size_t)b * TILE;
        r.step = (size_t)G * TILE;
        r.nfull = full_tiles > b ? (full_tiles - b + G - 1) / G : 0;
        r.tail_base = (size_t)full_tiles * TILE;
        r.tail_count = (b == full_tiles % G) ? (unsigned)(N - r.tail_base) : 0;
    }
    return r;
}

extern __shared__ __attribute__((aligned(16))) double s_dyn_charge[];

template <int BLOCK, int UNROLL, int NT_STORE, bool FAULT = false, int EARLYZ = 0>
__global__ __launch_bounds__(BLOCK) void cavity_persistent_kernel(AosInputT<2> in, unsigned N, double Lx, double Ly, double Lz,
                                                                  DeviceParams prm, int L_typeid, SyncState st,
                                                                  uint64_t sequence, cavmd_result* __restrict__ res,
                                                                  HostResult* __restrict__ res_host,
                                                                  v2d* __restrict__ force2, unsigned lds_slots, int balanced)
{
    constexpr unsigned TILE = BLOCK * UNROLL;
    constexpr int MU = 2 * UNROLL;
    __shared__ double s_m[5];
    __shared__ int s_mi[3];
    double* s_charge = s_dyn_charge;
    const unsigned G = gridDim.x, b = blockIdx.x, tid = threadIdx.x;

    CAVMD_PSTAMP(0);
    if constexpr (FAULT)
    {
        if ((int)b == st.late_block)
        {
            const unsigned long long t0 = wall_clock64();
            while (wall_clock64() - t0 < (unsigned long long)st.late_ticks)
                __builtin_amdgcn_s_sleep(64);
        }
    }
    const unsigned tag = __hip_atomic_load(st.epoch, __ATOMIC_RELAXED, __HIP_MEMORY_SCOPE_AGENT);
    const unsigned nonce = ((unsigned)((uintptr_t)__builtin_amdgcn_dispatch_ptr() >> 6) * 2654435761u
                            ^ (unsigned)sequence * 40503u) | 1u;
    const unsigned poison = __hip_atomic_load(st.epoch + 2, __ATOMIC_RELAXED, __HIP_MEMORY_SCOPE_AGENT);
    const bool poisoned = poison != 0u && poison != nonce;
    const PhotonRow guess = photon_row(in, (size_t)(N - 1));

    Accum acc;
    const BlockRange rg = block_range<TILE>(N, G, b, balanced);
    for (unsigned slot = 0; slot < rg.nfull; ++slot)
    {
        const size_t base = rg.first + (size_t)slot * rg.step + tid;
        TileRegs<AosInputT<2>, UNROLL> A;
        tile_load<AosInputT<2>, BLOCK, UNROLL>(in, base, A);
        __builtin_amdgcn_sched_barrier(0);
        if (slot < lds_slots)
        {
#pragma unroll
            for (int u = 0; u < UNROLL; ++u)
                s_charge[slot * TILE + u * BLOCK + tid] = A.raw[u].c;
        }
        tile_accumulate<AosInputT<2>, BLOCK, UNROLL>(A, base, Lx, Ly, Lz, L_typeid, acc);
    }
    if (rg.tail_count)
    {
        const size_t base = rg.tail_base + tid;
#pragma unroll
        for (int u = 0; u < UNROLL; ++u)
        {
            const unsigned o = u * BLOCK + tid;
            double c = 0.0;
            if (o < rg.tail_count)
            {
                const size_t i = base + (size_t)u * BLOCK;
                const typename AosInputT<2>::Raw r = in.load(i);
                const double rx = AosInputT<2>::x(r) + (double)r.ix * Lx;
                const double ry = AosInputT<2>::y(r) + (double)r.iy * Ly;
                const double rz = AosInputT<2>::z(r) + (double)r.iz * Lz;
                acc.add((unsigned)i, rx, ry, rz, r.c, AosInputT<2>::tag(r), L_typeid);
                c = r.c;
            }
            if (rg.nfull < lds_slots)
                s_charge[rg.nfull * TILE + o] = c;
        }
    }
    CAVMD_PSTAMP(1);
    acc = block_reduce<BLOCK>(acc);
    CAVMD_PSTAMP(2);

    __shared__ __attribute__((aligned(8))) unsigned s_words[kGroup * kGranulesPerRecord];
    unsigned long long* const block_slab = st.granules;
    unsigned long long* const group_slab = st.granules + (size_t)kMaxPersistGrid * kGranulesPerRecord;
    if constexpr (EARLYZ != 0)
    {
        constexpr unsigned ZW = BLOCK / kWave - 1;
        if (tid >= kWave)
        {
            const unsigned w = tid / kWave - 1, lane = tid % kWave;
            const v2d z = {0.0, 0.0};
            for (unsigned slot = w; slot < rg.nfull; slot += ZW)
            {
                v2d* const f = force2 + 2 * (rg.first + (size_t)slot * rg.step) + 1;
#pragma unroll
                for (unsigned j = 0; j < TILE / kWave; ++j)
                    store_chunk<(EARLYZ == 2 ? 1 : 0)>(f + 2 * (size_t)(j * kWave + lane), z);
            }
            if (rg.tail_count && w == rg.nfull % ZW)
            {
                v2d* const f = force2 + 2 * rg.tail_base + 1;
                for (unsigned o = lane; o < rg.tail_count; o += kWave)
                    store_chunk<(EARLYZ == 2 ? 1 : 0)>(f + 2 * (size_t)o, z);
            }
        }
    }
    if (tid < kWave)
    {
        bool ok = !poisoned;
        bool silent = false;
#ifdef CAVMD_FAULT_SILENT_BLOCK
        silent = (b == CAVMD_FAULT_SILENT_BLOCK);
#endif
        if constexpr (FAULT)
            silent = silent || ((int)b == st.silent_block);
        if (!silent && !poisoned)
            publish_record(block_slab, kMaxPersistGrid, 1, b, tag, acc, s_words);
        Accum o, t;
        if (poisoned)
        {
        }
        else if (G <= (unsigned)kGroup)
        {
            ok = gather_records(block_slab, 0, G, tag, s_words, o, st.spin_limit, (int)b, acc, st.epoch + 1);
            CAVMD_PSTAMP(7);
        }
        else
        {
            if ((b & (kGroup - 1)) == 0)
            {
                const unsigned count = min(G - b, (unsigned)kGroup);
                Accum o1, t1;
                ok = gather_records(block_slab, b, count, tag, s_words, o1, st.spin_limit, 0, acc);
                if (ok)
                {
                    t1.merge(o1);
                    t1 = row_fold16(t1);
                    publish_record(group_slab, kGroup, kGroupCopies, b / kGroup, tag, t1, s_words);
                }
            }
            CAVMD_PSTAMP(7);
            ok = gather_records(group_slab + (size_t)(b % kGroupCopies) * kGroup * kGranulesPerRecord, 0,
                                (G + kGroup - 1) / kGroup, tag, s_words, o, st.spin_limit, -1, acc, st.epoch + 1)
                 && ok;
        }
        t.merge(o);
        const Accum tot = row_fold16(t);
        CAVMD_PSTAMP(3);
        const bool publisher = (b == G - 1);
        const Scalars sc = scalars_from_total<AosInputT<2>>(tot, guess, in, N, Lx, Ly, Lz, prm, publisher);
        if (tid == 0)
        {
            s_m[0] = sc.Dq[0]; s_m[1] = sc.Dq[1]; s_m[2] = sc.f[0]; s_m[3] = sc.f[1]; s_m[4] = sc.f[2];
            s_mi[0] = sc.photon;
            s_mi[1] = sc.nL;
            s_mi[2] = !ok;
            if (publisher && ok)
            {
                __hip_atomic_store(st.epoch, tag + 1u ? tag + 1u : 1u, __ATOMIC_RELAXED, __HIP_MEMORY_SCOPE_AGENT);
                write_result(res, sc, N, G, sequence);
                publish_to_host(res_host, sc, N, G, sequence);
            }
        }
    }
    CAVMD_PSTAMP(4);
    __syncthreads();
    CAVMD_PSTAMP(5);
    MapScalars m;
    m.Dqx = s_m[0]; m.Dqy = s_m[1]; m.Fx = s_m[2]; m.Fy = s_m[3]; m.Fz = s_m[4];
    m.photon = s_mi[0];
    m.nL = s_mi[1];
    const bool bad = s_mi[2];

    const size_t nchunks = 2 * (size_t)N;
    const v2d zero = {0.0, 0.0};
    auto slow_map = [&](unsigned t0, unsigned step, bool poison, const MapScalars& ms) {
        const double nan = __builtin_nan("");
        const double ng = -prm.g;
        const bool odd = tid & 1;
        for (unsigned t = t0; (size_t)t * TILE < N; t += step)
        {
#pragma unroll
            for (int u = 0; u < MU; ++u)
            {
                const size_t k = (size_t)t * 2 * TILE + (size_t)u * BLOCK + tid;
                if (k >= nchunks)
                    continue;
                v2d v = zero;
                if (poison)
                    v = (v2d) {nan, nan};
                else if (ms.photon >= 0)
                {
                    const size_t p = k >> 1;
                    const int ptag = __double2loint(in.pos2[2 * p + 1].y);
                    const double s = ng * in.charge[p];
                    v = (v2d) {s * ms.Dqx, s * ms.Dqy};
                    v = (odd || ptag == L_typeid) ? zero : v;
                    if (p == (size_t)ms.photon)
                        v = odd ? (v2d) {ms.Fz, 0.0} : (v2d) {ms.Fx, ms.Fy};
                }
                store_chunk<NT_STORE>(force2 + k, v);
            }
        }
    };
    if (bad)
    {
        __shared__ unsigned s_last;
        slow_map(b, G, true, m);
        __threadfence();
        __syncthreads();
        if (tid == 0)
        {
            __hip_atomic_store(st.sync_error, kSyncFailed, __ATOMIC_RELAXED, __HIP_MEMORY_SCOPE_SYSTEM);
            __hip_atomic_store(&res_host->failed, (sequence << 2) | kSyncFailed, __ATOMIC_RELAXED, __HIP_MEMORY_SCOPE_SYSTEM);
            if (poisoned)
                s_last = 0u;
            else
            {
                __hip_atomic_store(st.epoch + 2, nonce, __ATOMIC_RELAXED, __HIP_MEMORY_SCOPE_AGENT);
                s_last = __hip_atomic_fetch_add(st.epoch + 1, 1u, __ATOMIC_ACQ_REL, __HIP_MEMORY_SCOPE_AGENT) == G - 1;
            }
        }
        __syncthreads();
        if (!s_last)
            return;
        __shared__ __attribute__((aligned(8))) unsigned s_groups[kGroup * kGranulesPerRecord];
        if (tid < kWave)
        {
            bool ok = true;
            Accum o, t;
            if (G <= (unsigned)kGroup)
                ok = gather_records(block_slab, 0, G, tag, s_words, o, kRepairRounds, -1, acc);
            else
            {
                const unsigned ngroups = (G + kGroup - 1) / kGroup;
                for (unsigned g = 0; g < ngroups; ++g)
                {
                    Accum o1, t1;
                    ok = gather_records(block_slab, g * kGroup, min(G - g * kGroup, (unsigned)kGroup), tag, s_words, o1,
                                        kRepairRounds, -1, acc)
                         && ok;
                    t1.merge(o1);
                    t1 = row_fold16(t1);
                    if (tid == 0)
                        record_to_lds(s_groups + g * kGranulesPerRecord, t1);
                }
                if (tid < ngroups)
                    record_from_lds(s_groups + tid * kGranulesPerRecord, o);
            }
            t.merge(o);
            const Accum tot = row_fold16(t);
            const Scalars sc = scalars_from_total<AosInputT<2>>(tot, guess, in, N, Lx, Ly, Lz, prm, true);
            if (tid == 0)
            {
                s_m[0] = sc.Dq[0]; s_m[1] = sc.Dq[1]; s_m[2] = sc.f[0]; s_m[3] = sc.f[1]; s_m[4] = sc.f[2];
                s_mi[0] = sc.photon;
                s_mi[1] = sc.nL;
                s_mi[2] = !ok;
                if (ok)
                {
                    __hip_atomic_store(st.sync_error, kSyncRepaired, __ATOMIC_RELAXED, __HIP_MEMORY_SCOPE_SYSTEM);
                    write_result(res, sc, N, G, sequence);
                    publish_to_host(res_host, sc, N, G, sequence);
                }
            }
        }
        __syncthreads();
        MapScalars mr;
        mr.Dqx = s_m[0]; mr.Dqy = s_m[1]; mr.Fx = s_m[2]; mr.Fy = s_m[3]; mr.Fz = s_m[4];
        mr.photon = s_mi[0];
        mr.nL = s_mi[1];
        if (!s_mi[2])
            slow_map(0, 1, false, mr);
        if (tid == 0)
        {
            __hip_atomic_store(st.epoch + 1, 0u, __ATOMIC_RELAXED, __HIP_MEMORY_SCOPE_AGENT);
            __hip_atomic_store(st.epoch, tag + 1u ? tag + 1u : 1u, __ATOMIC_RELAXED, __HIP_MEMORY_SCOPE_AGENT);
            __hip_atomic_store(st.epoch + 2, 0u, __ATOMIC_RELAXED, __HIP_MEMORY_SCOPE_AGENT);
        }
        return;
    }
    if (m.photon < 0 || m.nL > 1)
    {
        slow_map(b, G, false, m);
        return;
    }

    const double ng = -prm.g;
    const size_t pchunk = 2 * (size_t)m.photon;
    if constexpr (EARLYZ != 0)
    {
        auto put = [&](size_t p, double c) {
            const double s = ng * c;
            v2d v = {s * m.Dqx, s * m.Dqy};
            if (p == (size_t)m.photon)
            {
                v = (v2d) {m.Fx, m.Fy};
                store_chunk<NT_STORE>(force2 + 2 * p + 1, (v2d) {m.Fz, 0.0});
            }
            store_chunk<NT_STORE>(force2 + 2 * p, v);
        };
        for (unsigned slot = 0; slot < rg.nfull; ++slot)
        {
            const size_t p0 = rg.first + (size_t)slot * rg.step + tid;
            double c[UNROLL];
#pragma unroll
            for (int u = 0; u < UNROLL; ++u)
                c[u] = slot < lds_slots ? s_charge[slot * TILE + u * BLOCK + tid]
                                        : __builtin_nontemporal_load(in.charge + p0 + (size_t)u * BLOCK);
#pragma unroll
            for (int u = 0; u < UNROLL; ++u)
                put(p0 + (size_t)u * BLOCK, c[u]);
        }
        if (rg.tail_count)
        {
#pragma unroll
            for (int u = 0; u < UNROLL; ++u)
            {
                const unsigned o = u * BLOCK + tid;
                if (o < rg.tail_count)
                    put(rg.tail_base + o, rg.nfull < lds_slots ? s_charge[rg.nfull * TILE + o] : in.charge[rg.tail_base + o]);
            }
        }
        CAVMD_PSTAMP(6);
        return;
    }
    const bool odd = tid & 1;
    auto store_tile = [&](unsigned slot, const double (&c)[MU]) {
        const size_t base = 2 * (rg.first + (size_t)slot * rg.step) + tid;
#pragma unroll
        for (int u = 0; u < MU; ++u)
        {
            const size_t k = base + (size_t)u * BLOCK;
            const double s = ng * c[u];
            v2d v = {s * m.Dqx, s * m.Dqy};
            v = odd ? zero : v;
            if ((k | 1) == (pchunk | 1))
                v = odd ? (v2d) {m.Fz, 0.0} : (v2d) {m.Fx, m.Fy};
            store_chunk<NT_STORE>(force2 + k, v);
        }
    };
    const unsigned resident = rg.nfull < lds_slots ? rg.nfull : lds_slots;
    for (unsigned slot = 0; slot < resident; ++slot)
    {
        double c[MU];
#pragma unroll
        for (int u = 0; u < MU; ++u)
            c[u] = s_charge[slot * TILE + ((u * BLOCK + tid) >> 1)];
        store_tile(slot, c);
    }
    if (resident < rg.nfull)
    {
        constexpr int D = 8;
        auto load_batch = [&](unsigned s0, double (&c)[D][MU]) {
#pragma unroll
            for (int d = 0; d < D; ++d)
            {
                const unsigned slot = s0 + d < rg.nfull ? s0 + d : rg.nfull - 1;
                const size_t p0 = rg.first + (size_t)slot * rg.step;
#pragma unroll
                for (int u = 0; u < MU; ++u)
                    c[d][u] = __builtin_nontemporal_load(in.charge + p0 + ((u * BLOCK + tid) >> 1));
            }
        };
        auto store_batch = [&](unsigned s0, const double (&c)[D][MU]) {
#pragma unroll
            for (int d = 0; d < D; ++d)
                if (s0 + d < rg.nfull)
                    store_tile(s0 + d, c[d]);
        };
        double A[D][MU], B[D][MU];
        load_batch(resident, A);
        for (unsigned s0 = resident; s0 < rg.nfull; s0 += 2 * D)
        {
            if (s0 + D < rg.nfull)
                load_batch(s0 + D, B);
            store_batch(s0, A);
            if (s0 + 2 * D < rg.nfull)
                load_batch(s0 + 2 * D, A);
            if (s0 + D < rg.nfull)
                store_batch(s0 + D, B);
        }
    }
    if (rg.tail_count)
    {
        const size_t base = 2 * rg.tail_base + tid;
#pragma unroll
        for (int u = 0; u < MU; ++u)
        {
            const unsigned o = (u * BLOCK + tid) >> 1;
            if (o < rg.tail_count)
            {
                const size_t k = base + (size_t)u * BLOCK;
                const double cc = rg.nfull < lds_slots ? s_charge[rg.nfull * TILE + o] : in.charge[rg.tail_base + o];
                const double s = ng * cc;
                v2d v = {s * m.Dqx, s * m.Dqy};
                v = odd ? zero : v;
                if ((k | 1) == (pchunk | 1))
                    v = odd ? (v2d) {m.Fz, 0.0} : (v2d) {m.Fx, m.Fy};
                store_chunk<NT_STORE>(force2 + k, v);
            }
        }
    }
    CAVMD_PSTAMP(6);
}

}
```

### cav-hoomd_amd/csrc/cavmd_reduce.hpp

```cpp
#pragma once

#include <hip/hip_runtime.h>
#include <limits.h>
#include <stdint.h>

#include "cavmd.h"

#pragma clang fp contract(off)

#ifndef CAVMD_STAMP
#define CAVMD_STAMP(k)
#endif

namespace cavmd
{

typedef double v2d __attribute__((ext_vector_type(2)));
typedef int v3i __attribute__((ext_vector_type(3)));

constexpr int kWave = 64;
constexpr int kNumPartDoubles = 9;
constexpr int kNumPartInts = 2;

__device__ __forceinline__ void dd_acc(double& hi, double& lo, double t)
{
#if defined(CAVMD_DIAG_ACC_COST)
#if CAVMD_DIAG_ACC_COST == 0
    hi += t;
    return;
#else
    {
        const double s2 = lo + t;
        const double b2 = s2 - lo;
        const double e2 = (lo - (s2 - b2)) + (t - b2);
        asm volatile("" ::"v"(s2), "v"(e2));
    }
#endif
#endif
    const double s = hi + t;
    const double bb = s - hi;
    const double e = (hi - (s - bb)) + (t - bb);
    hi = s;
    lo += e;
}
__device__ __forceinline__ void dd_merge(double& hi, double& lo, double ohi, double olo)
{
    const double s = hi + ohi;
    const double bb = s - hi;
    const double e = (hi - (s - bb)) + (ohi - bb);
    hi = s;
    lo = (lo + olo) + e;
}
__device__ __forceinline__ void dd_norm(double& hi, double& lo)
{
    const double s = hi + lo;
    const double bb = s - hi;
    const double e = (hi - (s - bb)) + (lo - bb);
    hi = s;
    lo = e;
}

template <int CTRL, int ROW_MASK>
__device__ __forceinline__ double dpp_f64(double v, double ident)
{
    const int lo = __builtin_amdgcn_update_dpp(__double2loint(ident), __double2loint(v), CTRL, ROW_MASK, 0xf, false);
    const int hi = __builtin_amdgcn_update_dpp(__double2hiint(ident), __double2hiint(v), CTRL, ROW_MASK, 0xf, false);
    return __hiloint2double(hi, lo);
}
template <int CTRL, int ROW_MASK>
__device__ __forceinline__ int dpp_i32(int v, int ident)
{
    return __builtin_amdgcn_update_dpp(ident, v, CTRL, ROW_MASK, 0xf, false);
}

struct Accum
{
    double hx = 0.0, lx = 0.0, hy = 0.0, ly = 0.0, hz = 0.0, lz = 0.0;
    double sx = 0.0, sy = 0.0, sz = 0.0;
    int lmin = INT_MAX;
    int lcnt = 0;

    __device__ __forceinline__ void add(unsigned idx, double rx, double ry, double rz, double c, int tag, int L_typeid)
    {
        const double tx = c * rx;
        const double ty = c * ry;
        const double tz = c * rz;
        const bool isL = (tag == L_typeid);
        dd_acc(hx, lx, isL ? 0.0 : tx);
        dd_acc(hy, ly, isL ? 0.0 : ty);
        dd_acc(hz, lz, isL ? 0.0 : tz);
        sx += isL ? tx : 0.0;
        sy += isL ? ty : 0.0;
        sz += isL ? tz : 0.0;
        lmin = isL ? min(lmin, (int)idx) : lmin;
        lcnt += isL ? 1 : 0;
    }
    __device__ __forceinline__ void merge(const Accum& o)
    {
        dd_merge(hx, lx, o.hx, o.lx);
        dd_merge(hy, ly, o.hy, o.ly);
        dd_merge(hz, lz, o.hz, o.lz);
        sx += o.sx;
        sy += o.sy;
        sz += o.sz;
        lmin = min(lmin, o.lmin);
        lcnt += o.lcnt;
    }
    template <int CTRL, int ROW_MASK>
    __device__ __forceinline__ void dpp_step(bool withL)
    {
        dd_merge(hx, lx, dpp_f64<CTRL, ROW_MASK>(hx, 0.0), dpp_f64<CTRL, ROW_MASK>(lx, 0.0));
        dd_merge(hy, ly, dpp_f64<CTRL, ROW_MASK>(hy, 0.0), dpp_f64<CTRL, ROW_MASK>(ly, 0.0));
        dd_merge(hz, lz, dpp_f64<CTRL, ROW_MASK>(hz, 0.0), dpp_f64<CTRL, ROW_MASK>(lz, 0.0));
        if (withL)
        {
            sx += dpp_f64<CTRL, ROW_MASK>(sx, 0.0);
            sy += dpp_f64<CTRL, ROW_MASK>(sy, 0.0);
            sz += dpp_f64<CTRL, ROW_MASK>(sz, 0.0);
            lmin = min(lmin, dpp_i32<CTRL, ROW_MASK>(lmin, INT_MAX));
            lcnt += dpp_i32<CTRL, ROW_MASK>(lcnt, 0);
        }
    }
};

struct DD
{
    double hi, lo;
};
__device__ __forceinline__ DD dd_sel(bool c, DD a, DD b)
{
    DD r;
    r.hi = c ? a.hi : b.hi;
    r.lo = c ? a.lo : b.lo;
    return r;
}
__device__ __forceinline__ DD dd_sum(DD a, DD b)
{
    dd_merge(a.hi, a.lo, b.hi, b.lo);
    return a;
}
template <int CTRL>
__device__ __forceinline__ DD dd_dpp(DD v)
{
    DD r;
    r.hi = dpp_f64<CTRL, 0xF>(v.hi, 0.0);
    r.lo = dpp_f64<CTRL, 0xF>(v.lo, 0.0);
    return r;
}
__device__ __forceinline__ DD dd_shfl_xor(DD v, int mask)
{
    DD r;
    r.hi = __shfl_xor(v.hi, mask, kWave);
    r.lo = __shfl_xor(v.lo, mask, kWave);
    return r;
}

template <int BLOCK>
__device__ __forceinline__ Accum block_reduce_generic(Accum a)
{
    constexpr int NW = BLOCK / kWave;
    __shared__ double s_d[NW][kNumPartDoubles];
    __shared__ int s_i[NW][kNumPartInts];
    const bool anyL = __any(a.lcnt != 0);
    a.dpp_step<0xB1, 0xF>(anyL);
    a.dpp_step<0x4E, 0xF>(anyL);
    a.dpp_step<0x141, 0xF>(anyL);
    a.dpp_step<0x140, 0xF>(anyL);
    a.dpp_step<0x142, 0xA>(anyL);
    a.dpp_step<0x143, 0xC>(anyL);
    CAVMD_STAMP(2);
    const int lane = threadIdx.x & (kWave - 1);
    const int wave = threadIdx.x / kWave;
    if (lane == kWave - 1)
    {
        s_d[wave][0] = a.hx; s_d[wave][1] = a.lx; s_d[wave][2] = a.hy; s_d[wave][3] = a.ly;
        s_d[wave][4] = a.hz; s_d[wave][5] = a.lz; s_d[wave][6] = a.sx; s_d[wave][7] = a.sy;
        s_d[wave][8] = a.sz;
        s_i[wave][0] = a.lmin;
        s_i[wave][1] = a.lcnt;
    }
    __syncthreads();
    if (threadIdx.x == 0)
    {
        a.hx = s_d[0][0]; a.lx = s_d[0][1]; a.hy = s_d[0][2]; a.ly = s_d[0][3];
        a.hz = s_d[0][4]; a.lz = s_d[0][5]; a.sx = s_d[0][6]; a.sy = s_d[0][7];
        a.sz = s_d[0][8];
        a.lmin = s_i[0][0];
        a.lcnt = s_i[0][1];
#pragma unroll
        for (int w = 1; w < NW; ++w)
        {
            Accum o;
            o.hx = s_d[w][0]; o.lx = s_d[w][1]; o.hy = s_d[w][2]; o.ly = s_d[w][3];
            o.hz = s_d[w][4]; o.lz = s_d[w][5]; o.sx = s_d[w][6]; o.sy = s_d[w][7];
            o.sz = s_d[w][8];
            o.lmin = s_i[w][0];
            o.lcnt = s_i[w][1];
            a.merge(o);
        }
    }
    CAVMD_STAMP(3);
    return a;
}

__device__ __forceinline__ Accum block_reduce_256(Accum a)
{
    constexpr int NW = 4;
    __shared__ double s_main[NW][4][2];
    __shared__ double s_L[NW][3];
    __shared__ int s_Li[NW][2];
    const int lane = threadIdx.x & (kWave - 1);
    const int wave = threadIdx.x / kWave;

    if (__any(a.lcnt != 0))
    {
#define CAVMD_L_STEP(CTRL, MASK)                                     \
    a.sx += dpp_f64<CTRL, MASK>(a.sx, 0.0);                          \
    a.sy += dpp_f64<CTRL, MASK>(a.sy, 0.0);                          \
    a.sz += dpp_f64<CTRL, MASK>(a.sz, 0.0);                          \
    a.lmin = min(a.lmin, dpp_i32<CTRL, MASK>(a.lmin, INT_MAX));      \
    a.lcnt += dpp_i32<CTRL, MASK>(a.lcnt, 0);
        CAVMD_L_STEP(0xB1, 0xF)
        CAVMD_L_STEP(0x4E, 0xF)
        CAVMD_L_STEP(0x141, 0xF)
        CAVMD_L_STEP(0x140, 0xF)
        CAVMD_L_STEP(0x142, 0xA)
        CAVMD_L_STEP(0x143, 0xC)
#undef CAVMD_L_STEP
    }

    const bool b0 = lane & 1, b1 = lane & 2;
    const DD X {a.hx, a.lx}, Y {a.hy, a.ly}, Z {a.hz, a.lz}, W {0.0, 0.0};
    const DD P = dd_sum(dd_sel(b0, Z, X), dd_dpp<0xB1>(dd_sel(b0, X, Z)));
    const DD Q = dd_sum(dd_sel(b0, W, Y), dd_dpp<0xB1>(dd_sel(b0, Y, W)));
    DD R = dd_sum(dd_sel(b1, Q, P), dd_dpp<0x4E>(dd_sel(b1, P, Q)));
    R = dd_sum(R, dd_dpp<0x124>(R));
    R = dd_sum(R, dd_dpp<0x128>(R));
    R = dd_sum(R, dd_shfl_xor(R, 16));
    R = dd_sum(R, dd_shfl_xor(R, 32));
    CAVMD_STAMP(2);

    if (lane < 4)
    {
        s_main[wave][lane][0] = R.hi;
        s_main[wave][lane][1] = R.lo;
    }
    if (lane == kWave - 1)
    {
        s_L[wave][0] = a.sx;
        s_L[wave][1] = a.sy;
        s_L[wave][2] = a.sz;
        s_Li[wave][0] = a.lmin;
        s_Li[wave][1] = a.lcnt;
    }
    __syncthreads();
    if (wave == 0)
    {
        DD T {0.0, 0.0};
        if (lane < 4 * NW)
        {
            T.hi = s_main[lane >> 2][lane & 3][0];
            T.lo = s_main[lane >> 2][lane & 3][1];
        }
        T = dd_sum(T, dd_dpp<0x124>(T));
        T = dd_sum(T, dd_dpp<0x128>(T));
        const DD Tz = dd_dpp<0x55>(T);
        const DD Ty = dd_dpp<0xAA>(T);
        a.hx = T.hi; a.lx = T.lo;
        a.hy = Ty.hi; a.ly = Ty.lo;
        a.hz = Tz.hi; a.lz = Tz.lo;
        if (lane == 0)
        {
            a.sx = s_L[0][0]; a.sy = s_L[0][1]; a.sz = s_L[0][2];
            a.lmin = s_Li[0][0];
            a.lcnt = s_Li[0][1];
#pragma unroll
            for (int w = 1; w < NW; ++w)
            {
                a.sx += s_L[w][0]; a.sy += s_L[w][1]; a.sz += s_L[w][2];
                a.lmin = min(a.lmin, s_Li[w][0]);
                a.lcnt += s_Li[w][1];
            }
        }
    }
    CAVMD_STAMP(3);
    return a;
}

__device__ __forceinline__ Accum row_fold16(Accum a)
{
    if (__any(a.lcnt != 0))
    {
#define CAVMD_L_STEP(CTRL)                                          \
    a.sx += dpp_f64<CTRL, 0xF>(a.sx, 0.0);                          \
    a.sy += dpp_f64<CTRL, 0xF>(a.sy, 0.0);                          \
    a.sz += dpp_f64<CTRL, 0xF>(a.sz, 0.0);                          \
    a.lmin = min(a.lmin, dpp_i32<CTRL, 0xF>(a.lmin, INT_MAX));      \
    a.lcnt += dpp_i32<CTRL, 0xF>(a.lcnt, 0);
        CAVMD_L_STEP(0xB1)
        CAVMD_L_STEP(0x4E)
        CAVMD_L_STEP(0x141)
        CAVMD_L_STEP(0x140)
#undef CAVMD_L_STEP
    }
    const int lane = threadIdx.x & (kWave - 1);
    const bool b0 = lane & 1, b1 = lane & 2;
    const DD X {a.hx, a.lx}, Y {a.hy, a.ly}, Z {a.hz, a.lz}, W {0.0, 0.0};
    const DD P = dd_sum(dd_sel(b0, Z, X), dd_dpp<0xB1>(dd_sel(b0, X, Z)));
    const DD Q = dd_sum(dd_sel(b0, W, Y), dd_dpp<0xB1>(dd_sel(b0, Y, W)));
    DD R = dd_sum(dd_sel(b1, Q, P), dd_dpp<0x4E>(dd_sel(b1, P, Q)));
    R = dd_sum(R, dd_dpp<0x124>(R));
    R = dd_sum(R, dd_dpp<0x128>(R));
    const DD Tz = dd_dpp<0x55>(R);
    const DD Ty = dd_dpp<0xAA>(R);
    a.hx = R.hi; a.lx = R.lo;
    a.hy = Ty.hi; a.ly = Ty.lo;
    a.hz = Tz.hi; a.lz = Tz.lo;
    return a;
}

template <int BLOCK>
__device__ __forceinline__ Accum block_reduce(Accum a)
{
    if constexpr (BLOCK == 256)
        return block_reduce_256(a);
    else
        return block_reduce_generic<BLOCK>(a);
}

}
```

### cav-hoomd_amd/csrc/microbench_persistent.hip

```cpp
#include <hip/hip_runtime.h>

#include <algorithm>
#include <cstdio>
#include <cstdlib>
#include <cstring>
#include <functional>
#include <random>
#include <string>
#include <vector>

#include "cavmd.h"

constexpr int kStampSlots = 8;
__device__ unsigned long long g_pstamps[4096 * kStampSlots];
__device__ unsigned g_xcc[4096];
#define CAVMD_PSTAMP(k)                                                \
    do                                                                 \
    {                                                                  \
        if (threadIdx.x == 0)                                          \
        {                                                              \
            g_pstamps[blockIdx.x * kStampSlots + (k)] = wall_clock64(); \
            if ((k) == 0)                                              \
                g_xcc[blockIdx.x] = __builtin_amdgcn_s_getreg(20 | (0 << 6) | (3 << 11)) & 0xF;  \
        }                                                              \
    } while (0)
#include "cavmd_kernels.hpp"

using namespace cavmd;

#define CHECK(x)                                                                          \
    do                                                                                    \
    {                                                                                     \
        hipError_t e_ = (x);                                                              \
        if (e_ != hipSuccess)                                                             \
        {                                                                                 \
            fprintf(stderr, "%s:%d %s -> %s\n", __FILE__, __LINE__, #x, hipGetErrorString(e_)); \
            exit(1);                                                                      \
        }                                                                                 \
    } while (0)

struct Variant
{
    std::string name;
    std::function<void(int frame)> launch;
    std::vector<double> us;
};

int main(int argc, char** argv)
{
    const size_t N = argc > 1 ? strtoull(argv[1], nullptr, 10) : 1000001;
    const int frames = argc > 2 ? atoi(argv[2]) : 7;
    const int rounds = argc > 3 ? atoi(argv[3]) : 9;
    const int per_round = argc > 4 ? atoi(argv[4]) : 20;
    hipDeviceProp_t prop;
    CHECK(hipGetDeviceProperties(&prop, 0));
    const int CU = prop.multiProcessorCount;
    printf("device %s, %d CUs; N=%zu frames=%d rounds=%d launches/round=%d\n", prop.gcnArchName, CU, N, frames, rounds,
           per_round);

    std::mt19937_64 rng(1234);
    std::uniform_real_distribution<double> U(-100.0, 100.0), C(-1.0, 1.0);
    std::vector<cavmd_double4> h_pos(N);
    std::vector<double> h_chg(N);
    std::vector<cavmd_int3> h_img(N);
    for (size_t i = 0; i < N; ++i)
    {
        h_pos[i].x = U(rng); h_pos[i].y = U(rng); h_pos[i].z = U(rng);
        uint64_t tag = (i == N - 1) ? 2 : (i & 1);
        memcpy(&h_pos[i].w, &tag, 8);
        h_chg[i] = (i == N - 1) ? 0.0 : C(rng);
        h_img[i].x = (int)(rng() % 5) - 2; h_img[i].y = (int)(rng() % 5) - 2; h_img[i].z = (int)(rng() % 5) - 2;
    }
    std::vector<cavmd_double4*> d_pos(frames), d_frc(frames);
    std::vector<double*> d_chg(frames);
    std::vector<cavmd_int3*> d_img(frames);
    char* slab = nullptr;
    size_t slab_off = 0;
    auto piece = [&](size_t bytes) { char* p = slab + slab_off; slab_off += (bytes + (2u << 20) - 1) & ~(size_t)((2u << 20) - 1); return p; };
    if (getenv("CAVMD_SLAB"))
        CHECK(hipMalloc((void**)&slab, (size_t)frames * (N * 84 + (8u << 20)) + (2u << 20)));
    for (int f = 0; f < frames; ++f)
    {
        if (slab)
        {
            d_pos[f] = (cavmd_double4*)piece(N * 32); d_frc[f] = (cavmd_double4*)piece(N * 32);
            d_chg[f] = (double*)piece(N * 8);          d_img[f] = (cavmd_int3*)piece(N * 12);
        }
        else
        {
        CHECK(hipMalloc((void**)&d_pos[f], N * 32)); CHECK(hipMalloc((void**)&d_frc[f], N * 32));
        CHECK(hipMalloc((void**)&d_chg[f], N * 8));  CHECK(hipMalloc((void**)&d_img[f], N * 12));
        }
        CHECK(hipMemcpy(d_pos[f], h_pos.data(), N * 32, hipMemcpyHostToDevice));
        CHECK(hipMemcpy(d_chg[f], h_chg.data(), N * 8, hipMemcpyHostToDevice));
        CHECK(hipMemcpy(d_img[f], h_img.data(), N * 12, hipMemcpyHostToDevice));
    }
    for (int f = 0; f < frames; ++f)
        printf("frame %d: pos %p  force %p  charge %p  image %p\n", f, (void*)d_pos[f], (void*)d_frc[f], (void*)d_chg[f], (void*)d_img[f]);
    const unsigned max_parts = CU * 16;
    double* d_part; int* d_ipart; cavmd_result* d_res; HostResult* d_hres;
    unsigned long long* d_gran; unsigned* d_epoch; unsigned* d_syncerr;
    CHECK(hipMalloc((void**)&d_part, sizeof(double) * kNumPartDoubles * max_parts));
    CHECK(hipMalloc((void**)&d_ipart, sizeof(int) * kNumPartInts * max_parts));
    CHECK(hipMalloc((void**)&d_res, sizeof(cavmd_result)));
    CHECK(hipMalloc((void**)&d_hres, sizeof(HostResult)));
    CHECK(hipMalloc((void**)&d_gran, sizeof(unsigned long long) * 2 * kGranulesPerRecord * kMaxPersistGrid));
    CHECK(hipMemset(d_gran, 0, sizeof(unsigned long long) * 2 * kGranulesPerRecord * kMaxPersistGrid));
    CHECK(hipMalloc((void**)&d_epoch, 16));
    const unsigned epoch_init[4] = {1u, 0u, 0u, 0u};
    CHECK(hipMemcpy(d_epoch, epoch_init, 16, hipMemcpyHostToDevice));
    CHECK(hipMalloc((void**)&d_syncerr, sizeof(unsigned)));
    CHECK(hipMemset(d_syncerr, 0, sizeof(unsigned)));
    Partials part {d_part, d_ipart, max_parts};
    SyncState sync {d_gran, d_epoch, kSpinLimit, -1, 0u, -1, d_syncerr};
    const double L = 215.4;
    const unsigned n = (unsigned)N;
    hipStream_t st = 0;
    DeviceParams P; P.g = 1e-3; P.K = 0.0091 * 0.0091; P.gK = P.g / P.K; P.g2K = P.g * P.g / P.K;

    auto in0 = [&](int f) { AosInput in; in.pos2 = (const v2d*)d_pos[f]; in.charge = d_chg[f]; in.image = (const int*)d_img[f]; return in; };
    auto in1 = [&](int f) { AosInputT<1> in; in.pos2 = (const v2d*)d_pos[f]; in.charge = d_chg[f]; in.image = (const int*)d_img[f]; return in; };
    auto in2 = [&](int f) { AosInputT<2> in; in.pos2 = (const v2d*)d_pos[f]; in.charge = d_chg[f]; in.image = (const int*)d_img[f]; return in; };
    auto grid = [&](size_t items, unsigned tile, int bpc) {
        size_t tiles = (items + tile - 1) / tile; size_t cap = (size_t)CU * bpc; return (unsigned)std::max<size_t>(1, std::min(tiles, cap)); };

    int unroll = 2;
    while (unroll > 1 && N / ((size_t)256 * unroll) < (size_t)CU * 5 / 4)
        unroll >>= 1;
    const bool nts = N >= 200000;
#define ALLOW1(UNR, NTS, EZ) CHECK(hipFuncSetAttribute(reinterpret_cast<const void*>(&cavity_persistent_kernel<256, UNR, NTS, false, EZ>), hipFuncAttributeMaxDynamicSharedMemorySize, 156 * 1024))
#define ALLOW(UNR, NTS) do { ALLOW1(UNR, NTS, 0); ALLOW1(UNR, NTS, 1); ALLOW1(UNR, NTS, 2); } while (0)
    ALLOW(1, false); ALLOW(1, true); ALLOW(2, false); ALLOW(2, true);
    CHECK(hipFuncSetAttribute(reinterpret_cast<const void*>(&cavity_persistent_kernel<512, 1, true>), hipFuncAttributeMaxDynamicSharedMemorySize, 156 * 1024));
    CHECK(hipFuncSetAttribute(reinterpret_cast<const void*>(&cavity_persistent_kernel<512, 2, true>), hipFuncAttributeMaxDynamicSharedMemorySize, 156 * 1024));

#if defined(CAVMD_FAULT_SILENT_BLOCK) || defined(CAVMD_FAULT_LATE_BLOCK)
    {
        std::vector<double> h_f(4 * N, 0.0), h_want(4 * N, 0.0);
        const unsigned g1 = grid(N, 256 * unroll, 1);
        const size_t tile = 256 * unroll;
        const size_t slots = ((N + tile - 1) / tile + g1 - 1) / g1;
        if (unroll == 2)
            hipLaunchKernelGGL((dipole_partials_kernel<AosInputT<1>, 256, 2, false>), dim3(g1), dim3(256), 0, st, in1(0), n, L, L, L, 2, part);
        else
            hipLaunchKernelGGL((dipole_partials_kernel<AosInputT<1>, 256, 1, false>), dim3(g1), dim3(256), 0, st, in1(0), n, L, L, L, 2, part);
        hipLaunchKernelGGL((force_map_aos_fused_kernel<256, 4, false>), dim3(grid(2 * N, 1024, 2)), dim3(256), 0, st, in0(0), n, g1, L, L, L, P, 2, part, 1ull, d_res, d_hres, (v2d*)d_frc[0], false);
        CHECK(hipDeviceSynchronize());
        cavmd_result want_res; CHECK(hipMemcpy(&want_res, d_res, sizeof(want_res), hipMemcpyDeviceToHost));
        CHECK(hipMemcpy(h_want.data(), d_frc[0], 32 * N, hipMemcpyDeviceToHost));
        CHECK(hipMemset(d_frc[0], 0x5A, 32 * N));
        CHECK(hipMemset(d_hres, 0, sizeof(HostResult)));
        CHECK(hipMemset(d_res, 0, sizeof(cavmd_result)));
        hipEvent_t a, b2;
        CHECK(hipEventCreate(&a)); CHECK(hipEventCreate(&b2));
        CHECK(hipEventRecord(a, st));
#ifdef CAVMD_FAULT_LATE_BLOCK
        SyncState fsync = sync;
        fsync.spin_limit = 20000;
        fsync.late_block = CAVMD_FAULT_LATE_BLOCK;
        fsync.late_ticks = 6000000;
        CHECK(hipFuncSetAttribute(reinterpret_cast<const void*>(&cavity_persistent_kernel<256, 2, true, true>), hipFuncAttributeMaxDynamicSharedMemorySize, 156 * 1024));
        CHECK(hipFuncSetAttribute(reinterpret_cast<const void*>(&cavity_persistent_kernel<256, 1, true, true>), hipFuncAttributeMaxDynamicSharedMemorySize, 156 * 1024));
        if (unroll == 2)
            hipLaunchKernelGGL((cavity_persistent_kernel<256, 2, true, true>), dim3(g1), dim3(256), slots * tile * 8, st, in2(0), n, L, L, L, P, 2, fsync, 7ull, d_res, d_hres, (v2d*)d_frc[0], (unsigned)slots, false);
        else
            hipLaunchKernelGGL((cavity_persistent_kernel<256, 1, true, true>), dim3(g1), dim3(256), slots * tile * 8, st, in2(0), n, L, L, L, P, 2, fsync, 7ull, d_res, d_hres, (v2d*)d_frc[0], (unsigned)slots, false);
#else
        if (unroll == 2)
            hipLaunchKernelGGL((cavity_persistent_kernel<256, 2, true>), dim3(g1), dim3(256), slots * tile * 8, st, in2(0), n, L, L, L, P, 2, sync, 7ull, d_res, d_hres, (v2d*)d_frc[0], (unsigned)slots, false);
        else
            hipLaunchKernelGGL((cavity_persistent_kernel<256, 1, true>), dim3(g1), dim3(256), slots * tile * 8, st, in2(0), n, L, L, L, P, 2, sync, 7ull, d_res, d_hres, (v2d*)d_frc[0], (unsigned)slots, false);
#endif
        CHECK(hipEventRecord(b2, st));
        CHECK(hipEventSynchronize(b2));
        float ms; CHECK(hipEventElapsedTime(&ms, a, b2));
        HostResult hr; CHECK(hipMemcpy(&hr, d_hres, sizeof(hr), hipMemcpyDeviceToHost));
        unsigned sync_error; CHECK(hipMemcpy(&sync_error, d_syncerr, sizeof(sync_error), hipMemcpyDeviceToHost));
        cavmd_result got_res; CHECK(hipMemcpy(&got_res, d_res, sizeof(got_res), hipMemcpyDeviceToHost));
        unsigned after[3]; CHECK(hipMemcpy(after, d_epoch, 12, hipMemcpyDeviceToHost));
        CHECK(hipMemcpy(h_f.data(), d_frc[0], 32 * N, hipMemcpyDeviceToHost));
        size_t nan = 0, differ = 0;
        for (size_t i = 0; i < h_f.size(); ++i) { nan += (h_f[i] != h_f[i]); differ += memcmp(&h_f[i], &h_want[i], 8) != 0; }
        const bool same_dipole = memcmp(got_res.dipole, want_res.dipole, sizeof(got_res.dipole)) == 0
                                 && memcmp(hr.result.dipole, want_res.dipole, sizeof(got_res.dipole)) == 0;
#ifdef CAVMD_FAULT_SILENT_BLOCK
        (void)differ; (void)same_dipole;
        printf("fault injection (block %d silent, grid %u): kernel returned after %.1f ms, sync_error=%u, ready=%llu, slot failure word %llu, NaN force entries %zu of %zu, epoch %u, give-up count left %u, poison word %s\n",
               CAVMD_FAULT_SILENT_BLOCK, g1, ms, sync_error, (unsigned long long)hr.ready, (unsigned long long)hr.failed, nan, h_f.size(), after[0], after[1], after[2] ? "set" : "clear");
        return (sync_error == 1 && hr.failed == ((7ull << 2) | kSyncFailed) && nan >= h_f.size() - 4 * (size_t)tile && hr.ready == 0) ? 0 : 1;
#else
        printf("fault injection (block %d late, grid %u): kernel returned after %.1f ms, sync_error=%u, ready=%llu, NaN force entries %zu, force entries differing from the two-launch path %zu of %zu, dipole identical %d, epoch %u, give-up count left %u, poison word %s\n",
               CAVMD_FAULT_LATE_BLOCK, g1, ms, sync_error, (unsigned long long)hr.ready, nan, differ, h_f.size(), (int)same_dipole, after[0], after[1], after[2] ? "set" : "clear");
        return (sync_error == 2 && nan == 0 && differ == 0 && hr.ready == 7 && same_dipole && after[0] == 2 && after[1] == 0 && after[2] == 0) ? 0 : 1;
#endif
    }
#endif
    std::vector<Variant> V;
    V.push_back({"two launches (K1 nt1 bpc1 | fused map u4 bpc2)", [&](int f) {
                     const unsigned g1 = grid(N, 256 * unroll, 1);
                     if (unroll == 2)
                         hipLaunchKernelGGL((dipole_partials_kernel<AosInputT<1>, 256, 2, false>), dim3(g1), dim3(256), 0, st, in1(f), n, L, L, L, 2, part);
                     else
                         hipLaunchKernelGGL((dipole_partials_kernel<AosInputT<1>, 256, 1, false>), dim3(g1), dim3(256), 0, st, in1(f), n, L, L, L, 2, part);
                     const unsigned g2 = grid(2 * N, 1024, 2);
                     if (nts)
                         hipLaunchKernelGGL((force_map_aos_fused_kernel<256, 4, true>), dim3(g2), dim3(256), 0, st, in0(f), n, g1, L, L, L, P, 2, part, 1ull, d_res, d_hres, (v2d*)d_frc[f], false);
                     else
                         hipLaunchKernelGGL((force_map_aos_fused_kernel<256, 4, false>), dim3(g2), dim3(256), 0, st, in0(f), n, g1, L, L, L, P, 2, part, 1ull, d_res, d_hres, (v2d*)d_frc[f], false);
                 }, {}});
    auto persist = [&](int f, int bpc, int balanced = 0, int earlyz = 0) {
        const unsigned g1 = grid(N, 256 * unroll, bpc);
        const size_t tile = 256 * unroll;
        size_t slots = ((N + tile - 1) / tile + g1 - 1) / g1;
        if (balanced == 1) { const size_t units = (N + 63) / 64; slots = (((units + g1 - 1) / g1) * 64 + tile - 1) / tile; }
        if (balanced == 2) slots = (N / tile) / g1 + 1;
        const size_t cap = (156 * 1024 - 1024) / (tile * 8);
        const unsigned lds_slots = (unsigned)std::min(slots, cap);
        const size_t lds = (size_t)lds_slots * tile * 8;
#define PL(UNR, NTS, EZ) hipLaunchKernelGGL((cavity_persistent_kernel<256, UNR, NTS, false, EZ>), dim3(g1), dim3(256), lds, st, in2(f), n, L, L, L, P, 2, sync, 1ull, d_res, d_hres, (v2d*)d_frc[f], lds_slots, balanced)
#define PLZ(UNR, NTS) do { if (earlyz == 0) PL(UNR, NTS, 0); else if (earlyz == 1) PL(UNR, NTS, 1); else PL(UNR, NTS, 2); } while (0)
        if (unroll == 2) { if (nts) PLZ(2, true); else PLZ(2, false); }
        else { if (nts) PLZ(1, true); else PLZ(1, false); }
    };
    V.push_back({"single launch, tiles dealt round-robin", [&](int f) { persist(f, 1, 0); }, {}});
    V.push_back({"single launch, balanced contiguous shares", [&](int f) { persist(f, 1, 1); }, {}});
    V.push_back({"single launch, full rounds strided + last round split evenly", [&](int f) { persist(f, 1, 2); }, {}});
    if (getenv("CAVMD_TRY_EARLYZ")) {
        V.push_back({"single launch, zero chunks early (plain stores)", [&](int f) { persist(f, 1, 0, 1); }, {}});
        V.push_back({"single launch, zero chunks early (nt stores)", [&](int f) { persist(f, 1, 0, 2); }, {}});
    }
    auto persist512 = [&](int f, int unr) {
        const size_t tile = 512 * unr;
        const unsigned g1 = grid(N, tile, 1);
        size_t slots = ((N + tile - 1) / tile + g1 - 1) / g1;
        const size_t cap = (156 * 1024 - 1024) / (tile * 8);
        const unsigned lds_slots = (unsigned)std::min(slots, cap);
        const size_t lds = (size_t)lds_slots * tile * 8;
        if (unr == 1) hipLaunchKernelGGL((cavity_persistent_kernel<512, 1, true>), dim3(g1), dim3(512), lds, st, in2(f), n, L, L, L, P, 2, sync, 1ull, d_res, d_hres, (v2d*)d_frc[f], lds_slots, false);
        else hipLaunchKernelGGL((cavity_persistent_kernel<512, 2, true>), dim3(g1), dim3(512), lds, st, in2(f), n, L, L, L, P, 2, sync, 1ull, d_res, d_hres, (v2d*)d_frc[f], lds_slots, false);
    };
    if (getenv("CAVMD_TRY_512")) {
        V.push_back({"single launch, 512 threads x 1", [&](int f) { persist512(f, 1); }, {}});
        V.push_back({"single launch, 512 threads x 2", [&](int f) { persist512(f, 2); }, {}});
    }

    {
        std::vector<double> want(4 * N), got(4 * N);
        for (size_t vi = 0; vi < V.size(); ++vi)
        {
            CHECK(hipMemset(d_frc[0], 0x5A, 32 * N));
            V[vi].launch(0);
            CHECK(hipDeviceSynchronize());
            CHECK(hipMemcpy((vi == 0 ? want : got).data(), d_frc[0], 32 * N, hipMemcpyDeviceToHost));
            if (vi > 0)
            {
                size_t differ = 0; double worst = 0;
                for (size_t i = 0; i < got.size(); ++i)
                {
                    differ += memcmp(&got[i], &want[i], 8) != 0;
                    const double d = got[i] - want[i], sc = want[i] < 0 ? -want[i] : want[i];
                    if (sc > 0 && (d < 0 ? -d : d) / sc > worst) worst = (d < 0 ? -d : d) / sc;
                }
                printf("check %-60s entries differing from two launches: %zu of %zu (worst relative %.1e)\n", V[vi].name.c_str(), differ, got.size(), worst);
            }
        }
    }
    hipEvent_t e0, e1;
    CHECK(hipEventCreate(&e0)); CHECK(hipEventCreate(&e1));
    int frame = 0;
    for (auto& v : V) for (int f = 0; f < frames; ++f) v.launch(f);
    CHECK(hipDeviceSynchronize());
    for (int r = 0; r < rounds; ++r)
    {
        for (auto& v : V)
        {
            CHECK(hipEventRecord(e0, st));
            for (int k = 0; k < per_round; ++k) { v.launch(frame); frame = (frame + 1) % frames; }
            CHECK(hipEventRecord(e1, st));
            CHECK(hipEventSynchronize(e1));
            float ms; CHECK(hipEventElapsedTime(&ms, e0, e1));
            v.us.push_back(1e3 * ms / per_round);
        }
    }
    CHECK(hipGetLastError());
    printf("%-52s %10s %10s %12s\n", "variant", "med us", "min us", "evals/s(med)");
    for (auto& v : V)
    {
        std::sort(v.us.begin(), v.us.end());
        const double med = v.us[v.us.size() / 2], mn = v.us.front();
        printf("%-52s %10.2f %10.2f %12.0f\n", v.name.c_str(), med, mn, 1e6 / med);
    }

    const int timeline_earlyz = getenv("CAVMD_TIMELINE_EARLYZ") ? atoi(getenv("CAVMD_TIMELINE_EARLYZ")) : 0;
    const int timeline_partition = getenv("CAVMD_TIMELINE_PARTITION") ? atoi(getenv("CAVMD_TIMELINE_PARTITION")) : 0;
    printf("time line of the variant with partition %d, EARLYZ %d\n", timeline_partition, timeline_earlyz);
    for (int mode = 0; mode < 1; ++mode)
    {
        const unsigned g1 = grid(N, 256 * unroll, 1);
        const char* names[8] = {"start", "phase1 done", "block tree done", "total in wave 0", "scalars in LDS",
                                "barrier passed", "stores issued", "group level done"};
        std::vector<std::vector<double>> med(8), mx(8), mnv(8);
        std::vector<std::vector<double>> xcc_p1(30, std::vector<double>(8, 0.0));
        std::vector<int> xcc_frame(30, 0);
        for (int rep = 0; rep < 30; ++rep)
        {
            for (int k = 0; k < 12; ++k) persist((rep + k) % frames, 1, timeline_partition, timeline_earlyz);
            CHECK(hipDeviceSynchronize());
            std::vector<unsigned long long> h(4096 * kStampSlots);
            CHECK(hipMemcpyFromSymbol(h.data(), HIP_SYMBOL(g_pstamps), sizeof(unsigned long long) * h.size()));
            unsigned long long t0 = ~0ull;
            for (unsigned b = 0; b < g1; ++b) t0 = std::min(t0, h[b * kStampSlots]);
            {
                std::vector<unsigned> hx(4096);
                CHECK(hipMemcpyFromSymbol(hx.data(), HIP_SYMBOL(g_xcc), sizeof(unsigned) * hx.size()));
                std::vector<double> sum(8, 0.0); std::vector<int> cnt(8, 0);
                for (unsigned b = 0; b < g1; ++b) { const unsigned x = hx[b] & 7; sum[x] += (double)(h[b * kStampSlots + 1] - t0) * 0.01; cnt[x]++; }
                for (int x = 0; x < 8; ++x) xcc_p1[rep][x] = cnt[x] ? sum[x] / cnt[x] : 0.0;
                xcc_frame[rep] = (rep + 11) % frames;
                if (rep == 29) { printf("  blocks per XCC_ID in the last run:"); for (int x = 0; x < 8; ++x) printf(" %d", cnt[x]); printf("\n"); }
            }
            if (rep == 29 && getenv("CAVMD_DUMP_BLOCKS"))
            {
                printf("  per block: b tiles start phase1_done tree_done\n");
                const unsigned full_tiles = (unsigned)(N / (256 * unroll));
                for (unsigned b = 0; b < g1; ++b)
                {
                    const unsigned nt = full_tiles > b ? (full_tiles - b + g1 - 1) / g1 : 0;
                    printf("  blk %3u %u %.2f %.2f %.2f\n", b, nt, (double)(h[b * kStampSlots] - t0) * 0.01,
                           (double)(h[b * kStampSlots + 1] - t0) * 0.01, (double)(h[b * kStampSlots + 2] - t0) * 0.01);
                }
            }
            if (rep == 29)
            {
                printf("  per blockIdx%%8 group (start / tree done / fold done, us): ");
                for (unsigned x = 0; x < 8; ++x)
                {
                    double a = 1e9, c = 0, d = 0; unsigned cnt = 0;
                    for (unsigned b = x; b < g1; b += 8) { a = std::min(a, (double)(h[b * kStampSlots] - t0) * 0.01); c = std::max(c, (double)(h[b * kStampSlots + 2] - t0) * 0.01); d += (double)(h[b * kStampSlots + 4] - t0) * 0.01; ++cnt; }
                    printf("[%u: %.2f %.2f %.2f] ", x, a, c, d / cnt);
                }
                printf("\n  blocks 0..15 start: ");
                for (unsigned b = 0; b < 16 && b < g1; ++b) printf("%.2f ", (double)(h[b * kStampSlots] - t0) * 0.01);
                printf("\n  blocks 0..15 fold done: ");
                for (unsigned b = 0; b < 16 && b < g1; ++b) printf("%.2f ", (double)(h[b * kStampSlots + 4] - t0) * 0.01);
                printf("\n");
            }
            for (int k = 0; k < 8; ++k)
            {
                std::vector<double> v(g1);
                for (unsigned b = 0; b < g1; ++b) v[b] = (double)(h[b * kStampSlots + k] - t0) * 0.01;
                std::sort(v.begin(), v.end());
                med[k].push_back(v[g1 / 2]); mx[k].push_back(v.back()); mnv[k].push_back(v.front());
            }
        }
        printf("  mean phase-1-done per XCC_ID (us), one row per run (12 back-to-back launches each, stamps of the last):\n");
        for (int rep = 0; rep < 30; ++rep) { printf("   run %2d (frame %d):", rep, xcc_frame[rep]); for (int x = 0; x < 8; ++x) printf(" %6.2f", xcc_p1[rep][x]); printf("\n"); }
        printf("time line, single launch, grid %u (us after the first block's start; median over 30 runs of the per-run min / median / max over blocks)\n",
               g1);
        for (int k : {0, 1, 2, 7, 3, 4, 5, 6})
        {
            std::sort(med[k].begin(), med[k].end()); std::sort(mx[k].begin(), mx[k].end()); std::sort(mnv[k].begin(), mnv[k].end());
            printf("  %-22s min %6.2f  median %6.2f  max %6.2f\n", names[k], mnv[k][15], med[k][15], mx[k][15]);
        }
    }
    return 0;
}
```

Baseline: 50300 evals/s.

## Group persistent-kernel cross-block handoff by XCD with L2-scope polling

Changes the single-launch persistent kernel's grid-wide reduction handoff. Blocks are now grouped by blockIdx % 8, matching the XCD round-robin dispatch, instead of contiguous groups of 16. Blocks running on their home XCD also publish to a workgroup-scope (L2-local) slab, so the group leader can poll it cheaply and only occasionally falls back to agent scope. The small-grid partial reduction in the multi-launch finalize is also reworked to do a single load plus a 32-wide fold. This aims to cut cross-die coherence latency in the inter-block synchronisation, at the cost of extra stores, more sync slab memory and reliance on the XCD-placement assumption.

Result: slower. 49320 evals/s (-2.0%).

```diff
diff --git a/cav-hoomd_amd/csrc/cavmd_capi.hip b/cav-hoomd_amd/csrc/cavmd_capi.hip
--- a/cav-hoomd_amd/csrc/cavmd_capi.hip
+++ b/cav-hoomd_amd/csrc/cavmd_capi.hip
@@ -86,6 +86,7 @@
     int debug_late_block = -1;
     int debug_late_ticks = 0;
     int debug_silent_block = -1;
+    int debug_foreign_every = 0;
     int debug_skip_publish = 0;
     MappedBlock<HostResult> h_scratch;
     uint64_t suspend_until = 0;
@@ -474,7 +475,7 @@
     if (e == hipSuccess)
         e = ws->d_result.alloc_zeroed(1);
     if (e == hipSuccess)
-        e = ws->d_granules.alloc_zeroed((size_t)2 * kGranulesPerRecord * kMaxPersistGrid);
+        e = ws->d_granules.alloc_zeroed(kSyncGranules);
     if (e == hipSuccess)
         e = ws->d_epoch.alloc(4);
     if (e == hipSuccess)
@@ -615,7 +616,7 @@
     {
         if (ws->sync_state_dirty)
         {
-            CAVMD_HIP_TRY(hipMemsetAsync(ws->d_granules.ptr, 0, sizeof(unsigned long long) * 2 * kGranulesPerRecord * kMaxPersistGrid, stream));
+            CAVMD_HIP_TRY(hipMemsetAsync(ws->d_granules.ptr, 0, sizeof(unsigned long long) * kSyncGranules, stream));
             CAVMD_HIP_TRY(hipMemsetAsync(ws->d_epoch.ptr + 1, 0, 2 * sizeof(unsigned), stream));
             ws->sync_state_dirty = false;
         }
@@ -623,13 +624,14 @@
         const AosInputT<2> inx {in.pos2, in.charge, in.image};
         const SyncState sync {ws->d_granules.ptr, ws->d_epoch.ptr,
                               ws->debug_spin_limit > 0 ? (unsigned)ws->debug_spin_limit : kSpinLimit, ws->debug_late_block,
-                              (unsigned)ws->debug_late_ticks, ws->debug_silent_block, &ws->h_ctl.dev->sync_error};
+                              (unsigned)ws->debug_late_ticks, ws->debug_silent_block, ws->debug_foreign_every,
+                              &ws->h_ctl.dev->sync_error};
         const auto launch = [&](auto kernel) {
             return ls.launch_lds(0, plan.lds_bytes, kernel, plan.g1, kPersistBlock, inx, n, Lx, Ly, Lz, dp, L_typeid, sync,
                                  ws->sequence, d_result, host_block(ws), force2, plan.lds_slots, plan.balanced);
         };
 #ifdef CAVMD_TEST_HOOKS
-        if (ws->debug_late_block >= 0 || ws->debug_silent_block >= 0)
+        if (ws->debug_late_block >= 0 || ws->debug_silent_block >= 0 || ws->debug_foreign_every > 0)
             st = with_constant(kUnrolls, plan.unroll, [&](auto u) {
                 return launch(&cavity_persistent_kernel<kPersistBlock, decltype(u)::value, 0, true>);
             });
@@ -1329,6 +1331,7 @@
     {"debug_late_block", &cavmd_workspace::debug_late_block, -1, (int)kMaxPersistGrid - 1},
     {"debug_late_ticks", &cavmd_workspace::debug_late_ticks, 0, 100000000},
     {"debug_silent_block", &cavmd_workspace::debug_silent_block, -1, (int)kMaxPersistGrid - 1},
+    {"debug_foreign_every", &cavmd_workspace::debug_foreign_every, 0, (int)kMaxPersistGrid},
 #endif
 };
 
diff --git a/cav-hoomd_amd/csrc/cavmd_force_kernels.hpp b/cav-hoomd_amd/csrc/cavmd_force_kernels.hpp
--- a/cav-hoomd_amd/csrc/cavmd_force_kernels.hpp
+++ b/cav-hoomd_amd/csrc/cavmd_force_kernels.hpp
@@ -331,39 +331,30 @@
 
     Accum acc;
     const unsigned s = part.stride;
-    constexpr int BATCH = 4;
-    for (unsigned base = 0; base < nparts; base += BATCH * BLOCK)
-    {
-        Accum o[BATCH];
-#pragma unroll
-        for (int j = 0; j < BATCH; ++j)
-        {
-            const unsigned p = base + j * BLOCK + threadIdx.x;
-            if (p < nparts)
-            {
-                o[j].hx = part.d[0 * s + p]; o[j].lx = part.d[1 * s + p];
-                o[j].hy = part.d[2 * s + p]; o[j].ly = part.d[3 * s + p];
-                o[j].hz = part.d[4 * s + p]; o[j].lz = part.d[5 * s + p];
-                o[j].sx = part.d[6 * s + p]; o[j].sy = part.d[7 * s + p]; o[j].sz = part.d[8 * s + p];
-                o[j].lmin = part.i[0 * s + p];
-                o[j].lcnt = part.i[1 * s + p];
-            }
-        }
-#pragma unroll
-        for (int j = 0; j < BATCH; ++j)
-            if (base + j * BLOCK < nparts)
-                acc.merge(o[j]);
-    }
-    CAVMD_STAMP(1);
+    const auto load_partial = [&](unsigned p, Accum& o) {
+        o.hx = part.d[0 * s + p]; o.lx = part.d[1 * s + p];
+        o.hy = part.d[2 * s + p]; o.ly = part.d[3 * s + p];
+        o.hz = part.d[4 * s + p]; o.lz = part.d[5 * s + p];
+        o.sx = part.d[6 * s + p]; o.sy = part.d[7 * s + p]; o.sz = part.d[8 * s + p];
+        o.lmin = part.i[0 * s + p];
+        o.lcnt = part.i[1 * s + p];
+    };
     if (BLOCK == 256 && nparts <= 256)
     {
-        __shared__ double s_gd[16][kNumPartDoubles];
-        __shared__ int s_gi[16][kNumPartInts];
-        acc = row_fold16(acc);
+        __shared__ double s_gd[8][kNumPartDoubles];
+        __shared__ int s_gi[8][kNumPartInts];
+        const bool one_group = nparts <= 16;
+        const unsigned p = one_group ? threadIdx.x : (threadIdx.x & 31) * 8 + (threadIdx.x >> 5);
+        Accum o;
+        if (p < nparts)
+            load_partial(p, o);
+        acc.merge(o);
+        CAVMD_STAMP(1);
+        acc = one_group ? row_fold16(acc) : pair_fold32(acc);
         CAVMD_STAMP(2);
-        if ((threadIdx.x & 15) == 0)
-        {
-            const int gidx = threadIdx.x >> 4;
+        if ((threadIdx.x & 31) == 0)
+        {
+            const int gidx = threadIdx.x >> 5;
             s_gd[gidx][0] = acc.hx; s_gd[gidx][1] = acc.lx; s_gd[gidx][2] = acc.hy; s_gd[gidx][3] = acc.ly;
             s_gd[gidx][4] = acc.hz; s_gd[gidx][5] = acc.lz; s_gd[gidx][6] = acc.sx; s_gd[gidx][7] = acc.sy;
             s_gd[gidx][8] = acc.sz;
@@ -373,24 +364,41 @@
         __syncthreads();
         if (threadIdx.x < kWave)
         {
-            Accum o;
-            if (threadIdx.x < (nparts + 15) / 16)
+            Accum g;
+            if (threadIdx.x < (one_group ? 1u : 8u))
             {
                 const int gidx = threadIdx.x;
-                o.hx = s_gd[gidx][0]; o.lx = s_gd[gidx][1]; o.hy = s_gd[gidx][2]; o.ly = s_gd[gidx][3];
-                o.hz = s_gd[gidx][4]; o.lz = s_gd[gidx][5]; o.sx = s_gd[gidx][6]; o.sy = s_gd[gidx][7];
-                o.sz = s_gd[gidx][8];
-                o.lmin = s_gi[gidx][0];
-                o.lcnt = s_gi[gidx][1];
+                g.hx = s_gd[gidx][0]; g.lx = s_gd[gidx][1]; g.hy = s_gd[gidx][2]; g.ly = s_gd[gidx][3];
+                g.hz = s_gd[gidx][4]; g.lz = s_gd[gidx][5]; g.sx = s_gd[gidx][6]; g.sy = s_gd[gidx][7];
+                g.sz = s_gd[gidx][8];
+                g.lmin = s_gi[gidx][0];
+                g.lcnt = s_gi[gidx][1];
             }
             Accum t;
-            t.merge(o);
+            t.merge(g);
             acc = row_fold16(t);
         }
         CAVMD_STAMP(3);
-    }
-    else
-        acc = block_reduce<BLOCK>(acc);
+        return scalars_from_total<Input>(acc, guess, in, N, Lx, Ly, Lz, prm, want_energies);
+    }
+    constexpr int BATCH = 4;
+    for (unsigned base = 0; base < nparts; base += BATCH * BLOCK)
+    {
+        Accum o[BATCH];
+#pragma unroll
+        for (int j = 0; j < BATCH; ++j)
+        {
+            const unsigned p = base + j * BLOCK + threadIdx.x;
+            if (p < nparts)
+                load_partial(p, o[j]);
+        }
+#pragma unroll
+        for (int j = 0; j < BATCH; ++j)
+            if (base + j * BLOCK < nparts)
+                acc.merge(o[j]);
+    }
+    CAVMD_STAMP(1);
+    acc = block_reduce<BLOCK>(acc);
     return scalars_from_total<Input>(acc, guess, in, N, Lx, Ly, Lz, prm, want_energies);
 }
 
diff --git a/cav-hoomd_amd/csrc/cavmd_persistent_kernel.hpp b/cav-hoomd_amd/csrc/cavmd_persistent_kernel.hpp
--- a/cav-hoomd_amd/csrc/cavmd_persistent_kernel.hpp
+++ b/cav-hoomd_amd/csrc/cavmd_persistent_kernel.hpp
@@ -16,7 +16,10 @@
 constexpr unsigned kRepairRounds = 4096;
 
 constexpr int kGroup = 16;
-constexpr unsigned kMaxPersistGrid = kGroup * kGroup;
+constexpr int kXcds = 8;
+constexpr int kGroupMax = 32;
+constexpr unsigned kMaxPersistGrid = kXcds * kGroupMax;
+constexpr unsigned kL2Burst = 3;
 #ifndef CAVMD_GROUP_COPIES
 #define CAVMD_GROUP_COPIES 8
 #endif
@@ -33,14 +36,25 @@
     int late_block;
     unsigned late_ticks;
     int silent_block;
+    int foreign_every;
     unsigned* sync_error;
 };
 constexpr unsigned kSyncFailed = 1u;
 constexpr unsigned kSyncRepaired = 2u;
 
+constexpr size_t kSyncGranules = (size_t)(2 * kMaxPersistGrid + kGroupCopies * kGroup) * kGranulesPerRecord;
+
 __device__ __forceinline__ unsigned long long granule_load(const unsigned long long* g)
 {
     return __hip_atomic_load(g, __ATOMIC_RELAXED, __HIP_MEMORY_SCOPE_AGENT);
+}
+template <int L2LOAD>
+__device__ __forceinline__ unsigned long long granule_load_l2(const unsigned long long* g)
+{
+    if constexpr (L2LOAD == 2)
+        return __builtin_nontemporal_load((const volatile unsigned long long*)g);
+    else
+        return __hip_atomic_load(g, __ATOMIC_RELAXED, __HIP_MEMORY_SCOPE_WORKGROUP);
 }
 
 __device__ __forceinline__ void record_to_lds(unsigned* s_rec, const Accum& a)
@@ -67,6 +81,7 @@
     o.lcnt = (int)w[19];
 }
 
+template <bool L2 = false>
 __device__ __forceinline__ void publish_record(unsigned long long* slab, unsigned slab_records, unsigned copies, unsigned rec,
                                                unsigned tag, const Accum& a, unsigned* s_pub)
 {
@@ -76,27 +91,47 @@
     const unsigned field = lane % kGranulesPerRecord, copy0 = lane / kGranulesPerRecord;
     const unsigned long long granule = ((unsigned long long)tag << 32) | s_pub[field];
     for (unsigned c = copy0; c < copies && copy0 < 3; c += 3)
-        __hip_atomic_store(slab + ((size_t)c * slab_records + rec) * kGranulesPerRecord + field, granule, __ATOMIC_RELAXED,
-                           __HIP_MEMORY_SCOPE_AGENT);
-}
-
+    {
+        unsigned long long* const g = slab + ((size_t)c * slab_records + rec) * kGranulesPerRecord + field;
+        if constexpr (L2)
+            __hip_atomic_store(g, granule, __ATOMIC_RELAXED, __HIP_MEMORY_SCOPE_WORKGROUP);
+        else
+            __hip_atomic_store(g, granule, __ATOMIC_RELAXED, __HIP_MEMORY_SCOPE_AGENT);
+    }
+}
+
+template <int MAXREC, int L2LOAD = 1>
 __device__ __forceinline__ bool gather_records(const unsigned long long* slab, unsigned first, unsigned count, unsigned tag,
                                                unsigned* s_words, Accum& o, unsigned max_rounds, int own_slot,
-                                               const Accum& own, const unsigned* giveups = nullptr)
-{
-    constexpr int ROUNDS = (kGroup * kGranulesPerRecord + kWave - 1) / kWave;
+                                               const Accum& own, const unsigned* giveups = nullptr,
+                                               const unsigned long long* l2_slab = nullptr)
+{
+    constexpr int ROUNDS = (MAXREC * kGranulesPerRecord + kWave - 1) / kWave;
     const unsigned lane = threadIdx.x;
     const unsigned total = count * kGranulesPerRecord;
     const unsigned long long* g = slab + (size_t)first * kGranulesPerRecord;
+    const unsigned long long* g2 = l2_slab ? l2_slab + (size_t)first * kGranulesPerRecord : nullptr;
     unsigned long long x[ROUNDS];
     for (unsigned spins = 1;; ++spins)
     {
         const unsigned gone = giveups ? __hip_atomic_load(giveups, __ATOMIC_RELAXED, __HIP_MEMORY_SCOPE_AGENT) : 0u;
-#pragma unroll
-        for (int j = 0; j < ROUNDS; ++j)
-        {
-            const unsigned i = j * kWave + lane;
-            x[j] = granule_load(g + (i < total ? i : total - 1));
+        if (g2 && spins % (kL2Burst + 1) != 0)
+        {
+#pragma unroll
+            for (int j = 0; j < ROUNDS; ++j)
+            {
+                const unsigned i = j * kWave + lane;
+                x[j] = granule_load_l2<L2LOAD>(g2 + (i < total ? i : total - 1));
+            }
+        }
+        else
+        {
+#pragma unroll
+            for (int j = 0; j < ROUNDS; ++j)
+            {
+                const unsigned i = j * kWave + lane;
+                x[j] = granule_load(g + (i < total ? i : total - 1));
+            }
         }
         bool ok = true;
 #pragma unroll
@@ -176,7 +211,7 @@
 
 extern __shared__ __attribute__((aligned(16))) double s_dyn_charge[];
 
-template <int BLOCK, int UNROLL, int NT_STORE, bool FAULT = false, int EARLYZ = 0>
+template <int BLOCK, int UNROLL, int NT_STORE, bool FAULT = false, int EARLYZ = 0, int HANDOFF = 2>
 __global__ __launch_bounds__(BLOCK) void cavity_persistent_kernel(AosInputT<2> in, unsigned N, double Lx, double Ly, double Lz,
                                                                   DeviceParams prm, int L_typeid, SyncState st,
                                                                   uint64_t sequence, cavmd_result* __restrict__ res,
@@ -249,9 +284,12 @@
     acc = block_reduce<BLOCK>(acc);
     CAVMD_PSTAMP(2);
 
-    __shared__ __attribute__((aligned(8))) unsigned s_words[kGroup * kGranulesPerRecord];
+    __shared__ __attribute__((aligned(8))) unsigned s_words[(HANDOFF != 0 ? kGroupMax : kGroup) * kGranulesPerRecord];
     unsigned long long* const block_slab = st.granules;
-    unsigned long long* const group_slab = st.granules + (size_t)kMaxPersistGrid * kGranulesPerRecord;
+    unsigned long long* const l2_slab = st.granules + (size_t)kMaxPersistGrid * kGranulesPerRecord;
+    unsigned long long* const group_slab = st.granules + (size_t)2 * kMaxPersistGrid * kGranulesPerRecord;
+    Scalars sc;
+    bool publish = false;
     if constexpr (EARLYZ != 0)
     {
         constexpr unsigned ZW = BLOCK / kWave - 1;
@@ -283,58 +321,94 @@
 #endif
         if constexpr (FAULT)
             silent = silent || ((int)b == st.silent_block);
+        constexpr bool kByXcd = HANDOFF != 0;
+        constexpr int kL2Load = HANDOFF == 3 ? 2 : 1;
+        const unsigned slot = (!kByXcd || G <= (unsigned)kGroup) ? b : (b % kXcds) * kGroupMax + b / kXcds;
+        bool home = HANDOFF >= 2 && G > (unsigned)kGroup
+                    && (__builtin_amdgcn_s_getreg(20 | (0 << 6) | (3 << 11)) & 7u) == b % kXcds;
+        if constexpr (FAULT)
+            home = home && !(st.foreign_every > 0 && b % (unsigned)st.foreign_every == (unsigned)st.foreign_every - 1u);
         if (!silent && !poisoned)
-            publish_record(block_slab, kMaxPersistGrid, 1, b, tag, acc, s_words);
+        {
+            if (home)
+                publish_record<true>(l2_slab, kMaxPersistGrid, 1, slot, tag, acc, s_words);
+            publish_record(block_slab, kMaxPersistGrid, 1, slot, tag, acc, s_words);
+        }
         Accum o, t;
         if (poisoned)
         {
         }
         else if (G <= (unsigned)kGroup)
         {
-            ok = gather_records(block_slab, 0, G, tag, s_words, o, st.spin_limit, (int)b, acc, st.epoch + 1);
+            ok = gather_records<kGroup>(block_slab, 0, G, tag, s_words, o, st.spin_limit, (int)b, acc, st.epoch + 1);
             CAVMD_PSTAMP(7);
         }
-        else
+        else if constexpr (!kByXcd)
         {
             if ((b & (kGroup - 1)) == 0)
             {
                 const unsigned count = min(G - b, (unsigned)kGroup);
                 Accum o1, t1;
-                ok = gather_records(block_slab, b, count, tag, s_words, o1, st.spin_limit, 0, acc);
+                ok = gather_records<kGroup>(block_slab, b, count, tag, s_words, o1, st.spin_limit, 0, acc);
+                CAVMD_PSTAMP(8);
                 if (ok)
                 {
                     t1.merge(o1);
                     t1 = row_fold16(t1);
+                    CAVMD_PSTAMP(9);
                     publish_record(group_slab, kGroup, kGroupCopies, b / kGroup, tag, t1, s_words);
                 }
             }
             CAVMD_PSTAMP(7);
-            ok = gather_records(group_slab + (size_t)(b % kGroupCopies) * kGroup * kGranulesPerRecord, 0,
-                                (G + kGroup - 1) / kGroup, tag, s_words, o, st.spin_limit, -1, acc, st.epoch + 1)
+            ok = gather_records<kGroup>(group_slab + (size_t)(b % kGroupCopies) * kGroup * kGranulesPerRecord, 0,
+                                        (G + kGroup - 1) / kGroup, tag, s_words, o, st.spin_limit, -1, acc, st.epoch + 1)
+                 && ok;
+        }
+        else
+        {
+            if (b < (unsigned)kXcds)
+            {
+                const unsigned count = (G - b + kXcds - 1) / kXcds;
+                Accum o1, t1;
+                ok = gather_records<kGroupMax, kL2Load>(block_slab, b * kGroupMax, count, tag, s_words, o1, st.spin_limit, 0,
+                                                        acc, nullptr, home ? l2_slab : nullptr);
+                CAVMD_PSTAMP(8);
+                if (ok)
+                {
+                    t1.merge(o1);
+                    t1 = pair_fold32(t1);
+                    CAVMD_PSTAMP(9);
+                    publish_record(group_slab, kGroup, kGroupCopies, b, tag, t1, s_words);
+                }
+            }
+            CAVMD_PSTAMP(7);
+            ok = gather_records<kXcds>(group_slab + (size_t)(b % kGroupCopies) * kGroup * kGranulesPerRecord, 0, kXcds, tag,
+                                       s_words, o, st.spin_limit, -1, acc, st.epoch + 1)
                  && ok;
         }
         t.merge(o);
         const Accum tot = row_fold16(t);
         CAVMD_PSTAMP(3);
         const bool publisher = (b == G - 1);
-        const Scalars sc = scalars_from_total<AosInputT<2>>(tot, guess, in, N, Lx, Ly, Lz, prm, publisher);
+        sc = scalars_from_total<AosInputT<2>>(tot, guess, in, N, Lx, Ly, Lz, prm, publisher);
         if (tid == 0)
         {
             s_m[0] = sc.Dq[0]; s_m[1] = sc.Dq[1]; s_m[2] = sc.f[0]; s_m[3] = sc.f[1]; s_m[4] = sc.f[2];
             s_mi[0] = sc.photon;
             s_mi[1] = sc.nL;
             s_mi[2] = !ok;
-            if (publisher && ok)
-            {
-                __hip_atomic_store(st.epoch, tag + 1u ? tag + 1u : 1u, __ATOMIC_RELAXED, __HIP_MEMORY_SCOPE_AGENT);
-                write_result(res, sc, N, G, sequence);
-                publish_to_host(res_host, sc, N, G, sequence);
-            }
+            publish = publisher && ok;
         }
     }
     CAVMD_PSTAMP(4);
     __syncthreads();
     CAVMD_PSTAMP(5);
+    if (publish)
+    {
+        __hip_atomic_store(st.epoch, tag + 1u ? tag + 1u : 1u, __ATOMIC_RELAXED, __HIP_MEMORY_SCOPE_AGENT);
+        write_result(res, sc, N, G, sequence);
+        publish_to_host(res_host, sc, N, G, sequence);
+    }
     MapScalars m;
     m.Dqx = s_m[0]; m.Dqy = s_m[1]; m.Fx = s_m[2]; m.Fy = s_m[3]; m.Fz = s_m[4];
     m.photon = s_mi[0];
@@ -393,24 +467,35 @@
         __syncthreads();
         if (!s_last)
             return;
-        __shared__ __attribute__((aligned(8))) unsigned s_groups[kGroup * kGranulesPerRecord];
+        __shared__ __attribute__((aligned(8))) unsigned s_groups[(HANDOFF != 0 ? kXcds : kGroup) * kGranulesPerRecord];
         if (tid < kWave)
         {
             bool ok = true;
             Accum o, t;
             if (G <= (unsigned)kGroup)
-                ok = gather_records(block_slab, 0, G, tag, s_words, o, kRepairRounds, -1, acc);
+                ok = gather_records<kGroup>(block_slab, 0, G, tag, s_words, o, kRepairRounds, -1, acc);
             else
             {
-                const unsigned ngroups = (G + kGroup - 1) / kGroup;
+                const unsigned ngroups = HANDOFF != 0 ? (unsigned)kXcds : (G + kGroup - 1) / kGroup;
                 for (unsigned g = 0; g < ngroups; ++g)
                 {
                     Accum o1, t1;
-                    ok = gather_records(block_slab, g * kGroup, min(G - g * kGroup, (unsigned)kGroup), tag, s_words, o1,
-                                        kRepairRounds, -1, acc)
-                         && ok;
-                    t1.merge(o1);
-                    t1 = row_fold16(t1);
+                    if constexpr (HANDOFF != 0)
+                    {
+                        ok = gather_records<kGroupMax>(block_slab, g * kGroupMax, (G - g + kXcds - 1) / kXcds, tag, s_words, o1,
+                                                       kRepairRounds, -1, acc)
+                             && ok;
+                        t1.merge(o1);
+                        t1 = pair_fold32(t1);
+                    }
+                    else
+                    {
+                        ok = gather_records<kGroup>(block_slab, g * kGroup, min(G - g * kGroup, (unsigned)kGroup), tag, s_words,
+                                                    o1, kRepairRounds, -1, acc)
+                             && ok;
+                        t1.merge(o1);
+                        t1 = row_fold16(t1);
+                    }
                     if (tid == 0)
                         record_to_lds(s_groups + g * kGranulesPerRecord, t1);
                 }
@@ -419,7 +504,7 @@
             }
             t.merge(o);
             const Accum tot = row_fold16(t);
-            const Scalars sc = scalars_from_total<AosInputT<2>>(tot, guess, in, N, Lx, Ly, Lz, prm, true);
+            sc = scalars_from_total<AosInputT<2>>(tot, guess, in, N, Lx, Ly, Lz, prm, true);
             if (tid == 0)
             {
                 s_m[0] = sc.Dq[0]; s_m[1] = sc.Dq[1]; s_m[2] = sc.f[0]; s_m[3] = sc.f[1]; s_m[4] = sc.f[2];
diff --git a/cav-hoomd_amd/csrc/cavmd_reduce.hpp b/cav-hoomd_amd/csrc/cavmd_reduce.hpp
--- a/cav-hoomd_amd/csrc/cavmd_reduce.hpp
+++ b/cav-hoomd_amd/csrc/cavmd_reduce.hpp
@@ -319,6 +319,20 @@
     return a;
 }
 
+__device__ __forceinline__ Accum pair_fold32(Accum a)
+{
+    a = row_fold16(a);
+    Accum o;
+    o.hx = __shfl_xor(a.hx, 16, kWave); o.lx = __shfl_xor(a.lx, 16, kWave);
+    o.hy = __shfl_xor(a.hy, 16, kWave); o.ly = __shfl_xor(a.ly, 16, kWave);
+    o.hz = __shfl_xor(a.hz, 16, kWave); o.lz = __shfl_xor(a.lz, 16, kWave);
+    o.sx = __shfl_xor(a.sx, 16, kWave); o.sy = __shfl_xor(a.sy, 16, kWave); o.sz = __shfl_xor(a.sz, 16, kWave);
+    o.lmin = __shfl_xor(a.lmin, 16, kWave);
+    o.lcnt = __shfl_xor(a.lcnt, 16, kWave);
+    a.merge(o);
+    return a;
+}
+
 template <int BLOCK>
 __device__ __forceinline__ Accum block_reduce(Accum a)
 {
diff --git a/cav-hoomd_amd/csrc/microbench_persistent.hip b/cav-hoomd_amd/csrc/microbench_persistent.hip
--- a/cav-hoomd_amd/csrc/microbench_persistent.hip
+++ b/cav-hoomd_amd/csrc/microbench_persistent.hip
@@ -11,7 +11,7 @@
 
 #include "cavmd.h"
 
-constexpr int kStampSlots = 8;
+constexpr int kStampSlots = 12;
 __device__ unsigned long long g_pstamps[4096 * kStampSlots];
 __device__ unsigned g_xcc[4096];
 #define CAVMD_PSTAMP(k)                                                \
@@ -104,15 +104,15 @@
     CHECK(hipMalloc((void**)&d_ipart, sizeof(int) * kNumPartInts * max_parts));
     CHECK(hipMalloc((void**)&d_res, sizeof(cavmd_result)));
     CHECK(hipMalloc((void**)&d_hres, sizeof(HostResult)));
-    CHECK(hipMalloc((void**)&d_gran, sizeof(unsigned long long) * 2 * kGranulesPerRecord * kMaxPersistGrid));
-    CHECK(hipMemset(d_gran, 0, sizeof(unsigned long long) * 2 * kGranulesPerRecord * kMaxPersistGrid));
+    CHECK(hipMalloc((void**)&d_gran, sizeof(unsigned long long) * kSyncGranules));
+    CHECK(hipMemset(d_gran, 0, sizeof(unsigned long long) * kSyncGranules));
     CHECK(hipMalloc((void**)&d_epoch, 16));
     const unsigned epoch_init[4] = {1u, 0u, 0u, 0u};
     CHECK(hipMemcpy(d_epoch, epoch_init, 16, hipMemcpyHostToDevice));
     CHECK(hipMalloc((void**)&d_syncerr, sizeof(unsigned)));
     CHECK(hipMemset(d_syncerr, 0, sizeof(unsigned)));
     Partials part {d_part, d_ipart, max_parts};
-    SyncState sync {d_gran, d_epoch, kSpinLimit, -1, 0u, -1, d_syncerr};
+    SyncState sync {d_gran, d_epoch, kSpinLimit, -1, 0u, -1, 0, d_syncerr};
     const double L = 215.4;
     const unsigned n = (unsigned)N;
     hipStream_t st = 0;
@@ -131,6 +131,9 @@
 #define ALLOW1(UNR, NTS, EZ) CHECK(hipFuncSetAttribute(reinterpret_cast<const void*>(&cavity_persistent_kernel<256, UNR, NTS, false, EZ>), hipFuncAttributeMaxDynamicSharedMemorySize, 156 * 1024))
 #define ALLOW(UNR, NTS) do { ALLOW1(UNR, NTS, 0); ALLOW1(UNR, NTS, 1); ALLOW1(UNR, NTS, 2); } while (0)
     ALLOW(1, false); ALLOW(1, true); ALLOW(2, false); ALLOW(2, true);
+#define ALLOWH(UNR, NTS, H) CHECK(hipFuncSetAttribute(reinterpret_cast<const void*>(&cavity_persistent_kernel<256, UNR, NTS, false, 0, H>), hipFuncAttributeMaxDynamicSharedMemorySize, 156 * 1024))
+#define ALLOWHS(H) do { ALLOWH(1, false, H); ALLOWH(1, true, H); ALLOWH(2, false, H); ALLOWH(2, true, H); } while (0)
+    ALLOWHS(0); ALLOWHS(1); ALLOWHS(3);
     CHECK(hipFuncSetAttribute(reinterpret_cast<const void*>(&cavity_persistent_kernel<512, 1, true>), hipFuncAttributeMaxDynamicSharedMemorySize, 156 * 1024));
     CHECK(hipFuncSetAttribute(reinterpret_cast<const void*>(&cavity_persistent_kernel<512, 2, true>), hipFuncAttributeMaxDynamicSharedMemorySize, 156 * 1024));
 
@@ -208,7 +211,7 @@
                      else
                          hipLaunchKernelGGL((force_map_aos_fused_kernel<256, 4, false>), dim3(g2), dim3(256), 0, st, in0(f), n, g1, L, L, L, P, 2, part, 1ull, d_res, d_hres, (v2d*)d_frc[f], false);
                  }, {}});
-    auto persist = [&](int f, int bpc, int balanced = 0, int earlyz = 0) {
+    auto persist = [&](int f, int bpc, int balanced = 0, int earlyz = 0, int handoff = 2) {
         const unsigned g1 = grid(N, 256 * unroll, bpc);
         const size_t tile = 256 * unroll;
         size_t slots = ((N + tile - 1) / tile + g1 - 1) / g1;
@@ -218,13 +221,19 @@
         const unsigned lds_slots = (unsigned)std::min(slots, cap);
         const size_t lds = (size_t)lds_slots * tile * 8;
 #define PL(UNR, NTS, EZ) hipLaunchKernelGGL((cavity_persistent_kernel<256, UNR, NTS, false, EZ>), dim3(g1), dim3(256), lds, st, in2(f), n, L, L, L, P, 2, sync, 1ull, d_res, d_hres, (v2d*)d_frc[f], lds_slots, balanced)
-#define PLZ(UNR, NTS) do { if (earlyz == 0) PL(UNR, NTS, 0); else if (earlyz == 1) PL(UNR, NTS, 1); else PL(UNR, NTS, 2); } while (0)
+#define PLH(UNR, NTS, H) hipLaunchKernelGGL((cavity_persistent_kernel<256, UNR, NTS, false, 0, H>), dim3(g1), dim3(256), lds, st, in2(f), n, L, L, L, P, 2, sync, 1ull, d_res, d_hres, (v2d*)d_frc[f], lds_slots, balanced)
+#define PLZ(UNR, NTS) do { if (handoff == 0) PLH(UNR, NTS, 0); else if (handoff == 1) PLH(UNR, NTS, 1); else if (handoff == 3) PLH(UNR, NTS, 3); else if (earlyz == 0) PL(UNR, NTS, 0); else if (earlyz == 1) PL(UNR, NTS, 1); else PL(UNR, NTS, 2); } while (0)
         if (unroll == 2) { if (nts) PLZ(2, true); else PLZ(2, false); }
         else { if (nts) PLZ(1, true); else PLZ(1, false); }
     };
     V.push_back({"single launch, tiles dealt round-robin", [&](int f) { persist(f, 1, 0); }, {}});
-    V.push_back({"single launch, balanced contiguous shares", [&](int f) { persist(f, 1, 1); }, {}});
-    V.push_back({"single launch, full rounds strided + last round split evenly", [&](int f) { persist(f, 1, 2); }, {}});
+    V.push_back({"  hand-off 0: groups of 16, agent scope (rounds 2-3)", [&](int f) { persist(f, 1, 0, 0, 0); }, {}});
+    V.push_back({"  hand-off 1: groups by b % 8, agent scope", [&](int f) { persist(f, 1, 0, 0, 1); }, {}});
+    V.push_back({"  hand-off 3: groups by b % 8, L2 polls non-temporal", [&](int f) { persist(f, 1, 0, 0, 3); }, {}});
+    if (getenv("CAVMD_TRY_PARTITIONS")) {
+        V.push_back({"single launch, balanced contiguous shares", [&](int f) { persist(f, 1, 1); }, {}});
+        V.push_back({"single launch, full rounds strided + last round split evenly", [&](int f) { persist(f, 1, 2); }, {}});
+    }
     if (getenv("CAVMD_TRY_EARLYZ")) {
         V.push_back({"single launch, zero chunks early (plain stores)", [&](int f) { persist(f, 1, 0, 1); }, {}});
         V.push_back({"single launch, zero chunks early (nt stores)", [&](int f) { persist(f, 1, 0, 2); }, {}});
@@ -293,41 +302,47 @@
 
     const int timeline_earlyz = getenv("CAVMD_TIMELINE_EARLYZ") ? atoi(getenv("CAVMD_TIMELINE_EARLYZ")) : 0;
     const int timeline_partition = getenv("CAVMD_TIMELINE_PARTITION") ? atoi(getenv("CAVMD_TIMELINE_PARTITION")) : 0;
-    printf("time line of the variant with partition %d, EARLYZ %d\n", timeline_partition, timeline_earlyz);
-    for (int mode = 0; mode < 1; ++mode)
-    {
+    for (int timeline_handoff : {0, 2})
+    {
+        printf("time line of the variant with partition %d, EARLYZ %d, hand-off %d\n", timeline_partition, timeline_earlyz, timeline_handoff);
         const unsigned g1 = grid(N, 256 * unroll, 1);
-        const char* names[8] = {"start", "phase1 done", "block tree done", "total in wave 0", "scalars in LDS",
-                                "barrier passed", "stores issued", "group level done"};
-        std::vector<std::vector<double>> med(8), mx(8), mnv(8);
+        const char* names[10] = {"start", "phase1 done", "block tree done", "total in wave 0", "scalars in LDS",
+                                 "barrier passed", "stores issued", "group level done", "leader: group gathered", "leader: group folded"};
+        std::vector<std::vector<double>> med(10), mx(10), mnv(10);
         std::vector<std::vector<double>> xcc_p1(30, std::vector<double>(8, 0.0));
         std::vector<int> xcc_frame(30, 0);
         for (int rep = 0; rep < 30; ++rep)
         {
-            for (int k = 0; k < 12; ++k) persist((rep + k) % frames, 1, timeline_partition, timeline_earlyz);
+            for (int k = 0; k < 12; ++k) persist((rep + k) % frames, 1, timeline_partition, timeline_earlyz, timeline_handoff);
             CHECK(hipDeviceSynchronize());
             std::vector<unsigned long long> h(4096 * kStampSlots);
             CHECK(hipMemcpyFromSymbol(h.data(), HIP_SYMBOL(g_pstamps), sizeof(unsigned long long) * h.size()));
             unsigned long long t0 = ~0ull;
             for (unsigned b = 0; b < g1; ++b) t0 = std::min(t0, h[b * kStampSlots]);
-            {
-                std::vector<unsigned> hx(4096);
-                CHECK(hipMemcpyFromSymbol(hx.data(), HIP_SYMBOL(g_xcc), sizeof(unsigned) * hx.size()));
+            std::vector<unsigned> hx(4096);
+            CHECK(hipMemcpyFromSymbol(hx.data(), HIP_SYMBOL(g_xcc), sizeof(unsigned) * hx.size()));
+            {
                 std::vector<double> sum(8, 0.0); std::vector<int> cnt(8, 0);
                 for (unsigned b = 0; b < g1; ++b) { const unsigned x = hx[b] & 7; sum[x] += (double)(h[b * kStampSlots + 1] - t0) * 0.01; cnt[x]++; }
                 for (int x = 0; x < 8; ++x) xcc_p1[rep][x] = cnt[x] ? sum[x] / cnt[x] : 0.0;
                 xcc_frame[rep] = (rep + 11) % frames;
-                if (rep == 29) { printf("  blocks per XCC_ID in the last run:"); for (int x = 0; x < 8; ++x) printf(" %d", cnt[x]); printf("\n"); }
+                if (rep == 29)
+                {
+                    printf("  blocks per XCC_ID in the last run:"); for (int x = 0; x < 8; ++x) printf(" %d", cnt[x]);
+                    unsigned on = 0; for (unsigned b = 0; b < g1; ++b) on += (hx[b] & 7) == b % 8;
+                    printf("; blocks with XCC_ID == blockIdx %% 8: %u of %u\n", on, g1);
+                }
             }
             if (rep == 29 && getenv("CAVMD_DUMP_BLOCKS"))
             {
-                printf("  per block: b tiles start phase1_done tree_done\n");
+                printf("  per block: b xcc tiles start phase1_done tree_done group_level_done total scalars barrier stores_issued\n");
                 const unsigned full_tiles = (unsigned)(N / (256 * unroll));
                 for (unsigned b = 0; b < g1; ++b)
                 {
                     const unsigned nt = full_tiles > b ? (full_tiles - b + g1 - 1) / g1 : 0;
-                    printf("  blk %3u %u %.2f %.2f %.2f\n", b, nt, (double)(h[b * kStampSlots] - t0) * 0.01,
-                           (double)(h[b * kStampSlots + 1] - t0) * 0.01, (double)(h[b * kStampSlots + 2] - t0) * 0.01);
+                    printf("  blk %3u %u %u", b, hx[b] & 7, nt);
+                    for (int k : {0, 1, 2, 7, 3, 4, 5, 6}) printf(" %.2f", (double)(h[b * kStampSlots + k] - t0) * 0.01);
+                    printf("\n");
                 }
             }
             if (rep == 29)
@@ -345,20 +360,23 @@
                 for (unsigned b = 0; b < 16 && b < g1; ++b) printf("%.2f ", (double)(h[b * kStampSlots + 4] - t0) * 0.01);
                 printf("\n");
             }
-            for (int k = 0; k < 8; ++k)
-            {
-                std::vector<double> v(g1);
-                for (unsigned b = 0; b < g1; ++b) v[b] = (double)(h[b * kStampSlots + k] - t0) * 0.01;
+            for (int k = 0; k < 10; ++k)
+            {
+                const unsigned nb = k < 8 ? g1 : std::min(g1, timeline_handoff ? 8u : (g1 + 15) / 16);
+                const unsigned stride = k < 8 ? 1 : (timeline_handoff ? 1 : 16);
+                std::vector<double> v(nb);
+                for (unsigned i = 0; i < nb; ++i) { const unsigned b = i * stride; v[i] = (double)(h[b * kStampSlots + k] - t0) * 0.01; }
                 std::sort(v.begin(), v.end());
-                med[k].push_back(v[g1 / 2]); mx[k].push_back(v.back()); mnv[k].push_back(v.front());
+                med[k].push_back(v[nb / 2]); mx[k].push_back(v.back()); mnv[k].push_back(v.front());
             }
         }
         printf("  mean phase-1-done per XCC_ID (us), one row per run (12 back-to-back launches each, stamps of the last):\n");
         for (int rep = 0; rep < 30; ++rep) { printf("   run %2d (frame %d):", rep, xcc_frame[rep]); for (int x = 0; x < 8; ++x) printf(" %6.2f", xcc_p1[rep][x]); printf("\n"); }
         printf("time line, single launch, grid %u (us after the first block's start; median over 30 runs of the per-run min / median / max over blocks)\n",
                g1);
-        for (int k : {0, 1, 2, 7, 3, 4, 5, 6})
-        {
+        for (int k : {0, 1, 2, 8, 9, 7, 3, 4, 5, 6})
+        {
+            if (k >= 8 && g1 <= 16) continue;
             std::sort(med[k].begin(), med[k].end()); std::sort(mx[k].begin(), mx[k].end()); std::sort(mnv[k].begin(), mnv[k].end());
             printf("  %-22s min %6.2f  median %6.2f  max %6.2f\n", names[k], mnv[k][15], med[k][15], mx[k][15]);
         }
```
